# dfyz/osm-renderer

Measured on AMD Instinct MI355X. Metric: tiles/sec (256x256 z=15), higher is better.
Workload: dtype f64; 1 GPU; BASELINE.json configs[1]: batch of 1024 z=15 256x256 tiles per GPU, synthetic 50-poly/200-segment geometry per tile (SplitMix64, SURVEY.md 8(d)), lat/lon f64 input resident in HBM, RGBA8 framebuffers written to HBM; 2 batches in flight (step i on resident copy / stream i mod 2: the pre-pass of one batch overlaps the raster stage of the previous one); tiles_this_rank=1024, polygons_per_tile=50, polylines_per_tile=40, scale=1, named_config=True, collective=none (1 GPU), rccl_nranks_seen=1, batches_in_flight=2

## Files before the change

osm_renderer_amd/build.py:

```python
import os
import shutil
import subprocess

HERE = os.path.dirname(os.path.abspath(__file__))
CSRC = os.path.join(HERE, "csrc")
LIB = os.path.join(HERE, "libosmtile.so")
SOURCES = ["osmt_kernels.hip", "osmt_labels.hip", "osmt_glyphs.hip", "osmt_textplace.hip", "osmt_textshape.hip", "osmt_polylabel.hip", "osmt_styled.hip", "osmt_tilequery.hip", "osmt_tilelabels.hip", "osmt_arealabels.hip", "osmt_selmatch.hip", "osmt_labelbind.hip", "osmt_cascade.hip", "osmt_anchors.hip", "osmt_pngenc.hip", "osmt_api.cpp", "osmt_png.cpp"]
HEADERS = ["osmt_bitonic.h", "osmt_cascade_rule.h", "osmt_cascade_tables.h", "osmt_geom.h", "osmt_glyph.h", "osmt_internal.h", "osmt_list_slices.h", "osmt_numparse.h", "osmt_png_table.h", "osmt_prebin_roles.h", "osmt_project.h", "osmt_utf8.h", os.path.join("..", "host", "osmt_textplacer.hpp"),
           os.path.join("..", "host", "osmt_textshaper.hpp"),
           os.path.join("..", "..", "include", "osmtile.h")]
LIBS = ["-lz", "-ldl", "-lpthread", "-Wl,--no-undefined"]
FLAGS = ["--offload-arch=gfx950", "-O3", "-std=c++17", "-ffp-contract=off", "-fPIC", "-shared", "-Wall"]


def _hipcc():
    for cand in (shutil.which("hipcc"), "/opt/rocm/bin/hipcc"):
        if cand and os.path.exists(cand):
            return cand
    raise RuntimeError("hipcc not found; libosmtile.so cannot be built")


def needs_build():
    if not os.path.exists(LIB):
        return True
    t = os.path.getmtime(LIB)
    deps = [os.path.join(CSRC, s) for s in SOURCES + HEADERS]
    return any(os.path.getmtime(d) > t for d in deps)


def build_variant(name, defines):
    out = os.path.join(HERE, f"libosmtile_{name}.so")
    cmd = [_hipcc()] + FLAGS + [f"-D{d}" for d in defines] + ["-o", out] + [os.path.join(CSRC, s) for s in SOURCES] + LIBS
    subprocess.check_call(cmd)
    return out


def build(force=False, verbose=False):
    if not force and not needs_build():
        return LIB
    cmd = [_hipcc()] + FLAGS + ["-o", LIB] + [os.path.join(CSRC, s) for s in SOURCES] + LIBS
    if verbose:
        print(" ".join(cmd))
    subprocess.check_call(cmd)
    return LIB


if __name__ == "__main__":
    print(build(force=True, verbose=True))
```

osm_renderer_amd/csrc/osmt_api.cpp:

```cpp
#include <hip/hip_runtime.h>

#include <algorithm>
#include <chrono>
#include <atomic>
#include <cmath>
#include <cstdarg>
#include <cstdio>
#include <cstring>
#include <condition_variable>
#include <deque>
#include <functional>
#include <map>
#include <dlfcn.h>

#include <memory>
#include <mutex>
#include <thread>
#include <new>
#include <string>
#include <vector>

#include "../../include/osmtile.h"
#include "osmt_cascade_tables.h"
#include "osmt_geom.h"
// ... 55 lines not shown
        uint64_t tick;
    };
    std::mutex cache_mu;
    std::vector<cached_buf> cache;
    uint64_t cache_tick = 0;
    std::vector<hipStream_t> idle_streams;
    hipStream_t poison_stream = nullptr;
    std::vector<cached_buf> host_cache;
    std::vector<osmt_image_desc> images;
    std::vector<double> image_pool_host;
    osmt_image_desc* d_images = nullptr;
    double4* d_image_pool = nullptr;
    uint32_t d_n_images = 0;
    std::vector<void*> image_graveyard;
    bool images_dirty = false;
    std::vector<osmt_glyph_vertex> glyph_verts;
    std::vector<uint32_t> glyph_voff{0u};
    osmt_glyph_vertex* d_glyph_verts = nullptr;
    uint32_t* d_glyph_voff = nullptr;
    uint32_t d_n_glyphs = 0;
    bool glyphs_dirty = false;
    struct font_host {
        std::vector<osmt_cmap_entry> cmap;
        std::vector<int32_t> advance;
        std::vector<uint32_t> outline;
        std::vector<osmt_kern_pair> kern;
        osmt_font_desc view{};
        void* d_pool = nullptr;
        osmt_font_dev dev{};
    };
    std::vector<std::shared_ptr<font_host>> fonts;
    osmt_font_dev* d_fonts = nullptr;
    uint32_t d_n_fonts = 0;
    bool fonts_dirty = false;
    struct geodata_host {
        size_t n_nodes = 0, n_ways = 0, n_mps = 0;
        void* d_pool = nullptr;
        osmt_geo_dev dev{};
        void* d_index = nullptr;
        osmt_tq_index_dev ix{};
        void* d_node_index = nullptr;
        const uint32_t *d_node_off = nullptr, *d_node_refs = nullptr, *d_zero_off = nullptr;
        const uint64_t* d_node_gid = nullptr;
        const double2* d_factors = nullptr;
        void* d_tags = nullptr;
        osmt_sm_tags_dev tags{};
        size_t tags_string_bytes = 0, n_node_tags = 0, n_way_tags = 0;
    };
    std::vector<geodata_host> geodata;
    struct selectors_host {
        void* d_pool = nullptr;
        osmt_sm_sels_dev dev{};
        std::shared_ptr<const std::vector<uint8_t>> zooms;
    };
    std::vector<selectors_host> selectors;
    struct rules_host {
        void* d_pool = nullptr;
        osmt_cs_rules_dev dev{};
        uint32_t selectors_id = 0;
        std::shared_ptr<const std::vector<uint32_t>> key_off;
        std::shared_ptr<const std::vector<uint8_t>> key_bytes;
    };
    std::vector<rules_host> rules;
    uint32_t match_hash_bits = 32;
    struct bindings_host {
        uint32_t geodata_id = 0;
        uint8_t zoom_lo = 0, zoom_hi = 0;
        void* d_pool = nullptr;
        osmt_tq_bind_dev dev{};
    };
    std::vector<bindings_host> bindings;
    struct label_bindings_host {
        uint32_t geodata_id = 0;
        uint8_t zoom_lo = 0, zoom_hi = 0;
        void* d_pool = nullptr;
        osmt_tl_bind_dev dev{};
        size_t n_nodes = 0, n_bindings = 0, n_texts = 0, n_chars = 0;
    };
    std::vector<label_bindings_host> label_bindings;
    struct area_label_bindings_host {
        uint32_t geodata_id = 0;
        uint8_t zoom_lo = 0, zoom_hi = 0;
        void* d_pool = nullptr;
        osmt_al_bind_dev dev{};
        size_t n_ways = 0, n_mps = 0, n_way_bindings = 0, n_mp_bindings = 0, n_texts = 0, n_chars = 0;
    };
    std::vector<area_label_bindings_host> area_label_bindings;
    std::vector<osmt_label_style_rec> label_styles;
    osmt_label_style_rec* d_label_styles = nullptr;
    uint32_t* d_label_rank = nullptr;
    uint32_t d_n_label_styles = 0;
    bool label_styles_dirty = false;
    std::vector<osmt_style_rec> styles;
    std::vector<double> style_dashes;
    osmt_style_rec* d_styles = nullptr;
    uint32_t* d_style_rank = nullptr;
    double* d_style_dashes = nullptr;
    uint32_t d_n_styles = 0;
    bool styles_dirty = false;
    std::atomic<int> refs{1};
    void* comm = nullptr;
    uint32_t comm_rank = 0, comm_size = 0;
    unsigned long long* d_count = nullptr;
    uint32_t* err_page = nullptr;
    std::vector<uint16_t> err_free;
    struct arena_density {
        double groups_per_fill = 0.0, recs_per_vseg = 0.0;
        uint32_t uploads = 0;
    } density[OSMT_MAX_SCALE + 1];
    std::mutex co_mu;
    std::condition_variable co_cv;
    std::deque<struct coalesce_req*> co_queue;
    int co_in_flight = 0;
    uint64_t pl_stats[3] = {0, 0, 0};
};

struct osmt_scene {
    osmt_ctx* ctx = nullptr;
    uint32_t n_jobs = 0, n_ops = 0, n_rings = 0, n_pts = 0, n_dashes = 0, n_strokes = 0;
    uint32_t scale = 1, coord_kind = 0, n_blk = 0;
    char* d_base = nullptr;
    char* d_front = nullptr;
    size_t bytes = 0;
    osmt_tile_job* d_jobs = nullptr;
    osmt_op* d_ops = nullptr;
    osmt_ring* d_rings = nullptr;
    double* d_latlon = nullptr;
    uint32_t* d_node_refs = nullptr;
    int32_t* d_pts = nullptr;
    double* d_dashes = nullptr;
    uint32_t* d_pt_job = nullptr;
    uint32_t* d_op_aux = nullptr;
    osmt_opinfo* d_info = nullptr;
    osmt_stroke_aux* d_aux = nullptr;
    osmt_dash_seg* d_dseg = nullptr;
    uint32_t* d_submask = nullptr;
    uint32_t* d_op_blk = nullptr;
    uint32_t* d_op_vseg = nullptr;
    osmt_blk_bbox* d_blk = nullptr;
    uint32_t* d_op_job = nullptr;
    osmt_vseg* d_vseg = nullptr;
    unsigned long long* d_cursors = nullptr;
    uint32_t* d_cnt = nullptr;
    uint2* d_hdr = nullptr;
    osmt_ent* d_ent = nullptr;
    unsigned long long ent_cap = 0;
    uint32_t n_fill_ops = 0;
    uint32_t n_vsegs = 0;
    char* d_arena = nullptr;
    uint32_t* d_fmask = nullptr;
    osmt_srec* d_srec = nullptr;
    uint2* d_skey = nullptr;
    unsigned long long fmask_cap = 0, srec_cap = 0;
    std::vector<uint32_t> h_pt_job, h_op_aux, h_op_blk, h_op_vseg, h_op_job, h_lab_wide;
    std::vector<osmt_label_band> h_lab_bands;
    std::vector<osmt_labelinfo> h_lab_info;
    hipStream_t own_stream = nullptr;
    std::mutex use_mu;
    std::vector<std::pair<hipStream_t, hipEvent_t>> last_use;
    void* h_stage = nullptr;
    uint32_t* h_err = nullptr;
    uint32_t max_job_ops = 0;
    bool arena_guess = false;
    uint32_t n_labels = 0, n_label_segs = 0;
    char* d_lab_base = nullptr;
    osmt_labelinfo* d_lab = nullptr;
    uint32_t* d_job_label_off = nullptr;
    double* d_lab_segs = nullptr;
    double* d_lab_a = nullptr;
    double* d_lab_s_wide = nullptr;
    uint32_t* d_lab_wide = nullptr;
    osmt_label_band* d_lab_bands = nullptr;
    unsigned long long* d_lab_bits = nullptr;
    uint32_t n_lab_bands = 0;
    uint32_t n_lab_wide = 0;
    bool lab_cover_valid = false;
    uint32_t* d_lab_bitmap = nullptr;
    uint8_t* d_lab_ok = nullptr;
    uint32_t* d_lab_err = nullptr;
    osmt_tile_label* d_tile_labels = nullptr;
    uint32_t* d_tile_label_cnt = nullptr;
    osmt_glyph_instance* d_text_inst = nullptr;
    uint32_t n_text_inst = 0;
    osmt_text_glyph* d_text_glyphs = nullptr;
    uint32_t n_text_glyphs = 0;
    char* d_tq = nullptr;
    char* d_tq_areas_buf = nullptr;
    const osmt_styled_tile* d_tq_tiles = nullptr;
    const osmt_styled_area* d_tq_areas = nullptr;
    size_t n_tq_areas = 0;
    std::vector<osmt_query_tile> h_tq_tiles;
    uint32_t tq_geodata_id = 0;
    std::vector<osmt_label> h_tl_labels;
    std::vector<osmt_string_run> h_tl_runs;
    std::vector<uint32_t> h_tl_chars, h_tl_off;
    std::vector<osmt_label> h_al_labels;
    std::vector<osmt_string_run> h_al_runs;
    std::vector<uint32_t> h_al_chars, h_al_off;
    std::vector<int32_t> h_al_pts;
    std::vector<double> h_al_sincos;
    std::vector<osmt_area_anchor> h_al_declined;
};

namespace {

constexpr double OSMT_MAX_ABS_LAT = 85.06;
size_t cache_keep_bytes() {
    static const size_t v = [] {
        const char* e = getenv("OSMT_CACHE_GB");
        const long gb = e ? atol(e) : 32;
        return (size_t)std::min<long>(std::max<long>(gb, 0), 256) << 30;
    }();
    return v;
}

bool poison_alloc() {
    static const bool v = [] {
        const char* e = getenv("OSMT_POISON_ALLOC");
        return e && *e && *e != '0';
    }();
    return v;
}

hipError_t stream_acquire(osmt_ctx* ctx, hipStream_t* out);
void stream_release(osmt_ctx* ctx, hipStream_t st);

hipError_t dev_poison(osmt_ctx* ctx, void* p, size_t bytes) {
    hipStream_t st = nullptr;
    {
        std::lock_guard<std::mutex> lk(ctx->cache_mu);
        if (!ctx->poison_stream) {
            int lo = 0, hi = 0;
            (void)hipDeviceGetStreamPriorityRange(&lo, &hi);
            if (hipStreamCreateWithPriority(&ctx->poison_stream, hipStreamNonBlocking, hi) != hipSuccess) {
                (void)hipGetLastError();
                ctx->poison_stream = nullptr;
            }
        }
        st = ctx->poison_stream;
    }
    const bool pooled = st == nullptr;
    hipError_t e = pooled ? stream_acquire(ctx, &st) : hipSuccess;
    if (e != hipSuccess) return e;
    e = hipMemsetAsync(p, 0xA5, bytes, st);
    if (e == hipSuccess) e = hipStreamSynchronize(st);
    if (pooled) stream_release(ctx, st);
    return e;
}

hipError_t dev_alloc_raw(osmt_ctx* ctx, void** out, size_t bytes, size_t* got);

hipError_t dev_alloc(osmt_ctx* ctx, void** out, size_t bytes) {
    size_t got = 0;
    hipError_t e = dev_alloc_raw(ctx, out, bytes, &got);
    if (e == hipSuccess && poison_alloc()) e = dev_poison(ctx, *out, got);
    return e;
}

hipError_t dev_alloc_raw(osmt_ctx* ctx, void** out, size_t bytes, size_t* got) {
    bytes = align_up(bytes ? bytes : 1, (size_t)2 << 20);
    {
        std::lock_guard<std::mutex> lk(ctx->cache_mu);
        osmt_ctx::cached_buf* best = nullptr;
        for (auto& c : ctx->cache)
            if (!c.used && c.bytes >= bytes && c.bytes <= 2 * bytes && (!best || c.bytes < best->bytes)) best = &c;
        if (best) {
            best->used = true;
            best->tick = ++ctx->cache_tick;
            *out = best->p;
            *got = best->bytes;
            return hipSuccess;
        }
    }
    hipError_t e = hipMalloc(out, bytes);
    if (e == hipErrorOutOfMemory) {
        (void)hipGetLastError();
        std::lock_guard<std::mutex> lk(ctx->cache_mu);
        for (size_t i = 0; i < ctx->cache.size();) {
            if (!ctx->cache[i].used) {
                (void)hipFree(ctx->cache[i].p);
                ctx->cache.erase(ctx->cache.begin() + (long)i);
            } else {
                ++i;
            }
        }
        e = hipMalloc(out, bytes);
    }
    if (e != hipSuccess) return e;
    std::lock_guard<std::mutex> lk(ctx->cache_mu);
    ctx->cache.push_back({*out, bytes, true, ++ctx->cache_tick});
    *got = bytes;
    return hipSuccess;
}

hipError_t stream_acquire(osmt_ctx* ctx, hipStream_t* out) {
    {
        std::lock_guard<std::mutex> lk(ctx->cache_mu);
        if (!ctx->idle_streams.empty()) {
            *out = ctx->idle_streams.back();
            ctx->idle_streams.pop_back();
            return hipSuccess;
        }
    }
    return hipStreamCreateWithFlags(out, hipStreamNonBlocking);
}

// ... 347 lines not shown
        if (e != hipSuccess && first == hipSuccess) first = e;
    }
    return first;
}

int validate_coords_range(const osmt_batch* b, size_t lo, size_t hi) {
    if (b->coord_kind == OSMT_COORD_POINT_I32) {
        for (size_t i = 2 * lo; i < 2 * hi; ++i)
            if (b->points[i] > OSMT_COORD_LIMIT || b->points[i] < -OSMT_COORD_LIMIT)
                return fail(OSMT_UNSUPPORTED, "point %zu: |coordinate| > 2^28", i / 2);
    } else {
        const double* ll = b->coord_kind == OSMT_COORD_NODE_REF ? b->nodes : b->latlon;
        for (size_t i = lo; i < hi; ++i) {
            const double lat = ll[2 * i], lon = ll[2 * i + 1];
            if (!(std::fabs(lat) <= OSMT_MAX_ABS_LAT) || !(std::fabs(lon) <= 180.0))
                return fail(OSMT_UNSUPPORTED, "point %zu: (lat, lon) = (%g, %g) outside the Web-Mercator square (|lat| <= %g, |lon| <= 180)", i, lat,
                            lon, OSMT_MAX_ABS_LAT);
        }
    }
    return OSMT_OK;
}
size_t coord_count(const osmt_batch* b) { return b->coord_kind == OSMT_COORD_NODE_REF ? b->n_nodes : b->n_pts; }

int validate_batch_global(const osmt_batch* b) {
    if (!b) return fail(OSMT_INVALID_ARG, "batch is NULL");
    if (b->scale < 1 || b->scale > OSMT_MAX_SCALE) return fail(OSMT_INVALID_ARG, "scale %u not in 1..%u", b->scale, OSMT_MAX_SCALE);
    if (b->coord_kind != OSMT_COORD_LATLON_F64 && b->coord_kind != OSMT_COORD_POINT_I32 && b->coord_kind != OSMT_COORD_NODE_REF)
        return fail(OSMT_INVALID_ARG, "unknown coord_kind %u", b->coord_kind);
    if (b->n_jobs >= 0x7FFFFFFFull / 64 || b->n_ops >= 0xFFFFFFFFull || b->n_rings >= 0xFFFFFFFFull ||
        b->n_pts >= 0xFFFFFFFFull || b->n_dashes >= 0xFFFFFFFFull)
        return fail(OSMT_INVALID_ARG, "batch too large for 32-bit indices");
    if ((b->n_jobs && !b->jobs) || (b->n_ops && !b->ops) || (b->n_rings && !b->rings) || (b->n_dashes && !b->dashes))
        return fail(OSMT_INVALID_ARG, "NULL pool with non-zero count");
    if (b->n_pts) {
        if (b->coord_kind == OSMT_COORD_LATLON_F64 && !b->latlon) return fail(OSMT_INVALID_ARG, "latlon pool is NULL");
        if (b->coord_kind == OSMT_COORD_POINT_I32 && !b->points) return fail(OSMT_INVALID_ARG, "points pool is NULL");
        if (b->coord_kind == OSMT_COORD_NODE_REF) {
            if (!b->node_refs || !b->nodes) return fail(OSMT_INVALID_ARG, "node table / node_refs is NULL");
            if (b->n_nodes >= 0xFFFFFFFFull) return fail(OSMT_INVALID_ARG, "node table too large for 32-bit indices");
        }
    }
    struct range {
        uint64_t lo, hi;
        uint32_t job;
    };
    std::vector<range> ops, pts;
    ops.reserve(b->n_jobs);
    pts.reserve(b->n_jobs);
    for (size_t j = 0; j < b->n_jobs; ++j) {
        const osmt_tile_job& job = b->jobs[j];
        if (job.zoom > OSMT_MAX_ZOOM) return fail(OSMT_INVALID_ARG, "job %zu: zoom %u > MAX_ZOOM (src/tile.rs:5)", j, job.zoom);
        if ((size_t)job.op_off + job.n_ops > b->n_ops) return fail(OSMT_INVALID_ARG, "job %zu: op range out of bounds", j);
        if ((size_t)job.pt_off + job.n_pts > b->n_pts) return fail(OSMT_INVALID_ARG, "job %zu: point range out of bounds", j);
        if (job.n_ops) ops.push_back({job.op_off, (uint64_t)job.op_off + job.n_ops, (uint32_t)j});
        if (job.n_pts) pts.push_back({job.pt_off, (uint64_t)job.pt_off + job.n_pts, (uint32_t)j});
    }
    auto by_lo = [](const range& x, const range& y) { return x.lo < y.lo; };
    std::sort(ops.begin(), ops.end(), by_lo);
    uint64_t next = 0;
    for (const range& r : ops) {
        if (r.lo < next)
            return fail(OSMT_INVALID_ARG, "job %u: op %llu also belongs to another job (op ranges must not overlap)", r.job, (unsigned long long)r.lo);
        if (r.lo > next)
            return fail(OSMT_INVALID_ARG, "op %llu is not covered by any job (the jobs' op ranges must partition the op pool)", (unsigned long long)next);
        next = r.hi;
    }
    if (next != b->n_ops)
        return fail(OSMT_INVALID_ARG, "op %llu is not covered by any job (the jobs' op ranges must partition the op pool)", (unsigned long long)next);
    std::sort(pts.begin(), pts.end(), by_lo);
    for (size_t i = 1; i < pts.size(); ++i)
        if (pts[i].lo < pts[i - 1].hi) return fail(OSMT_INVALID_ARG, "the point ranges of two jobs overlap at point %llu", (unsigned long long)pts[i].lo);
    return OSMT_OK;
}

int validate_job(const osmt_batch* b, size_t j, bool with_coords = true) {
    const osmt_tile_job& job = b->jobs[j];
    for (uint32_t k = 0; k < job.n_ops; ++k) {
        const osmt_op& op = b->ops[job.op_off + k];
        if (op.kind > OSMT_OP_STROKE) return fail(OSMT_INVALID_ARG, "job %zu op %u: unknown kind %u", j, k, op.kind);
        if (op.kind == OSMT_OP_NONE) continue;
        if ((size_t)op.ring_off + op.n_rings > b->n_rings) return fail(OSMT_INVALID_ARG, "job %zu op %u: ring range out of bounds", j, k);
        for (uint32_t r = 0; r < op.n_rings; ++r) {
            const osmt_ring& ring = b->rings[op.ring_off + r];
            if (ring.first_pt < job.pt_off || (size_t)ring.first_pt + ring.n_pts > (size_t)job.pt_off + job.n_pts)
                return fail(OSMT_INVALID_ARG, "job %zu op %u ring %u: points outside the job's pool range", j, k, r);
        }
        if (!(op.opacity >= 0.0) || !(op.opacity <= 4503599627370496.0))
            return fail(OSMT_INVALID_ARG, "job %zu op %u: opacity must be in [0, 2^52]", j, k);
        if (op.kind == OSMT_OP_STROKE) {
            if (!std::isfinite(op.width)) return fail(OSMT_INVALID_ARG, "job %zu op %u: width not finite", j, k);
            if (std::fabs(op.width) > 65536.0) return fail(OSMT_UNSUPPORTED, "job %zu op %u: |width| > 65536 px", j, k);
            if (op.cap > OSMT_CAP_SQUARE) return fail(OSMT_INVALID_ARG, "job %zu op %u: unknown cap", j, k);
            if (op.has_dashes) {
                if (op.n_dashes == 0) return fail(OSMT_INVALID_ARG, "job %zu op %u: empty dash list", j, k);
                if (op.n_dashes > OSMT_MAX_DASHES) return fail(OSMT_UNSUPPORTED, "job %zu op %u: more than %u dashes", j, k, OSMT_MAX_DASHES);
                if ((size_t)op.dashes_off + op.n_dashes > b->n_dashes) return fail(OSMT_INVALID_ARG, "job %zu op %u: dash range out of bounds", j, k);
            }
        }
    }
    if (b->coord_kind == OSMT_COORD_NODE_REF) {
        for (size_t i = job.pt_off; i < (size_t)job.pt_off + job.n_pts; ++i)
            if (b->node_refs[i] >= b->n_nodes) return fail(OSMT_INVALID_ARG, "point %zu: node reference %u out of range", i, b->node_refs[i]);
        return OSMT_OK;
    }
    return with_coords ? validate_coords_range(b, job.pt_off, (size_t)job.pt_off + job.n_pts) : OSMT_OK;
}

int validate_nodes(const osmt_batch* b, size_t lo, size_t hi) {
    return b->coord_kind == OSMT_COORD_NODE_REF ? validate_coords_range(b, lo, hi) : OSMT_OK;
}

int validate_batch(const osmt_batch* b, bool with_coords = true) {
    int rc = validate_batch_global(b);
    for (size_t j = 0; rc == OSMT_OK && j < b->n_jobs; ++j) rc = validate_job(b, j, with_coords);
    if (rc == OSMT_OK && with_coords) rc = validate_nodes(b, 0, b->n_nodes);
    return rc;
}

osmt_prepass_args prepass_args(const osmt_scene* sc, bool sizing) {
    osmt_prepass_args a;
    memset(&a, 0, sizeof a);
    a.jobs = sc->d_jobs;
    a.n_jobs = sc->n_jobs;
    a.ops = sc->d_ops;
    a.n_ops = sc->n_ops;
    a.rings = sc->d_rings;
    a.pts = reinterpret_cast<const int2*>(sc->d_pts);
    a.dashes = sc->d_dashes;
    a.op_aux = sc->d_op_aux;
    a.op_job = sc->d_op_job;
    a.op_blk = sc->d_op_blk;
    a.op_vseg = sc->d_op_vseg;
    a.vseg = sc->d_vseg;
    a.n_vsegs = sc->n_vsegs;
    a.max_job_ops = sc->max_job_ops;
    a.fold_max_ops = sc->n_jobs <= OSMT_FOLD_MAX_JOBS ? OSMT_FOLD_MAX_OPS : 0u;
    a.scale = sc->scale;
    a.sub_rows = OSMT_TILE_SIZE * sc->scale / OSMT_SUB_H;
    a.info = sc->d_info;
    a.aux = sc->d_aux;
    a.dseg = sc->d_dseg;
    a.blk = sc->d_blk;
    a.submask = sc->d_submask;
    a.cursors = sc->d_cursors;
    a.cnt = sc->d_cnt;
    a.hdr = sc->d_hdr;
    a.ent = sc->d_ent;
    a.ent_cap = sizing ? 0ull : sc->ent_cap;
    a.fmask = sc->d_fmask;
    a.srec = sc->d_srec;
    a.skey = sc->d_skey;
    a.fmask_cap = sizing ? 0ull : sc->fmask_cap;
    a.srec_cap = sizing ? 0ull : sc->srec_cap;
    a.err = sizing ? nullptr : sc->h_err;
    return a;
}

int render_impl(osmt_ctx* ctx, osmt_scene* sc, uint32_t stages, void* d_out, size_t stride, bool f64, void* stream,
                uint32_t first_job = 0, uint32_t n_range = 0) {
    if (!ctx || !sc || sc->ctx != ctx) return fail(OSMT_INVALID_ARG, "bad ctx/scene");
    HIP_TRY(hipSetDevice(ctx->device));
    hipStream_t st = (hipStream_t)stream;
    const uint32_t W = OSMT_TILE_SIZE * sc->scale;
    if ((stages & 4u) && !d_out) return fail(OSMT_INVALID_ARG, "output pointer is NULL");
    const bool rgb8 = (stages & 32u) != 0u;
    if ((stages & 4u) && !f64 && !rgb8 && stride < (size_t)W * W * 4) return fail(OSMT_INVALID_ARG, "out_tile_stride_bytes < W*H*4");
    if ((stages & 4u) && rgb8 && (f64 || stride < (size_t)W * W * 3 || (stride & 3u) || ((uintptr_t)d_out & 3u)))
        return fail(OSMT_INVALID_ARG, "RGB8 output: tile stride below W*H*3 or not a multiple of 4");
    bool zeroed = false;
    if ((stages & 1u) && sc->coord_kind != OSMT_COORD_POINT_I32) {
        const osmt_prepass_args pa = prepass_args(sc, false);
        zeroed = (stages & 2u) != 0u && sc->n_pts != 0u;
        HIP_TRY(osmt_launch_project(sc->d_jobs, sc->d_pt_job, sc->d_latlon, sc->coord_kind == OSMT_COORD_NODE_REF ? sc->d_node_refs : nullptr,
                                    sc->n_pts, (double)sc->scale, sc->d_pts, st, zeroed ? reinterpret_cast<uint32_t*>(pa.cursors) : nullptr,
                                    zeroed ? osmt_prepass_zero_words(pa) : 0));
    }
    if (stages & 2u) HIP_TRY(osmt_launch_prepass(prepass_args(sc, false), st, zeroed));
    const bool want_labels = sc->n_labels && !f64;
    if (want_labels && ((stages & 8u) || ((stages & 4u) && !(stages & 16u)))) {
        int rc = sync_images(ctx, nullptr);
        if (rc != OSMT_OK) return rc;
        osmt_label_launch ll;
        memset(&ll, 0, sizeof ll);
        ll.info = sc->d_lab;
        ll.n_labels = sc->n_labels;
        ll.n_jobs = sc->n_jobs;
        ll.scale = sc->scale;
        ll.n_wide = sc->n_lab_wide;
        ll.bands = sc->d_lab_bands;
        ll.n_bands = sc->n_lab_bands;
        ll.job_label_off = sc->d_job_label_off;
        ll.segs = sc->d_lab_segs;
        ll.wide = sc->d_lab_wide;
        ll.plane_a = sc->d_lab_a;
        ll.cell_bits = sc->d_lab_bits;
        ll.plane_s_wide = sc->d_lab_s_wide;
        ll.bitmap = sc->d_lab_bitmap;
        ll.ok = sc->d_lab_ok;
        ll.err = sc->d_lab_err;
        ll.tile_labels = sc->d_tile_labels;
        ll.tile_label_cnt = sc->d_tile_label_cnt;
        HIP_TRY(osmt_launch_labels(ll, st));
        sc->lab_cover_valid = true;
    }
    if (stages & 4u) {
        image_snapshot img;
        int rc = sync_images(ctx, &img);
        if (rc != OSMT_OK) return rc;
        if (first_job > sc->n_jobs || n_range > sc->n_jobs - first_job) return fail(OSMT_INVALID_ARG, "tile range out of bounds");
        const uint32_t n_render = n_range ? n_range : sc->n_jobs - first_job;
        osmt_raster_args a;
        memset(&a, 0, sizeof a);
        a.jobs = sc->d_jobs + first_job;
        a.n_jobs = n_render;
        a.scale = sc->scale;
        a.aux = sc->d_aux;
        a.dseg = sc->d_dseg;
        {
            const uint32_t Wt = OSMT_TILE_SIZE * sc->scale;
            a.hdr = sc->d_hdr + (size_t)first_job * (Wt / OSMT_SUB_W) * (Wt / OSMT_SUB_H);
        }
        a.ent = sc->d_ent;
        a.fmask = sc->d_fmask;
        a.srec = sc->d_srec;
        a.skey = sc->d_skey;
        a.info = sc->d_info;
        a.submask = sc->d_submask;
        a.fold_max_ops = sc->n_jobs <= OSMT_FOLD_MAX_JOBS ? OSMT_FOLD_MAX_OPS : 0u;
        a.images = img.desc;
        a.image_pool = img.pool;
        a.n_images = img.n;
        a.out = d_out;
        a.out_tile_stride = stride;
        a.out_rgb8 = rgb8 ? 1u : 0u;
        if (want_labels) {
            a.labels.info = sc->d_lab;
            a.labels.n_labels = sc->n_labels;
            a.labels.job_label_off = sc->d_job_label_off + first_job;
            a.labels.tile_labels = sc->d_tile_labels;
            a.labels.tile_label_cnt = sc->d_tile_label_cnt + first_job;
            a.labels.plane = sc->d_lab_a;
        }
        HIP_TRY(osmt_launch_raster(a, f64, st));
    }
    HIP_TRY(scene_mark_use(sc, st));
    return OSMT_OK;
}

}

extern "C" {

uint32_t osmt_version(void) { return (1u << 16) | 1u; }

const char* osmt_last_error(void) { return g_last_error.c_str(); }

static int osmt_create_body(const osmt_config* cfg, osmt_ctx** out_ctx) {
    if (!out_ctx) return fail(OSMT_INVALID_ARG, "out_ctx is NULL");
    *out_ctx = nullptr;
    int n = 0;
    hipError_t e = hipGetDeviceCount(&n);
    if (e != hipSuccess || n <= 0)
        return fail(OSMT_NO_DEVICE, "no HIP device available (%s); this library has no CPU path",
                    e == hipSuccess ? "device count 0" : hipGetErrorString(e));
    const int dev = cfg ? cfg->device : 0;
    if (dev < 0 || dev >= n) return fail(OSMT_INVALID_ARG, "device %d out of range (0..%d)", dev, n - 1);
    HIP_TRY(hipSetDevice(dev));
    osmt_ctx* c = new (std::nothrow) osmt_ctx();
    if (!c) return fail(OSMT_OOM, "out of host memory");
    c->device = dev;
    *out_ctx = c;
    return OSMT_OK;
}

int osmt_create(const osmt_config* cfg, osmt_ctx** out_ctx) {
    return guarded([&] { return osmt_create_body(cfg, out_ctx); });
}

void osmt_destroy(osmt_ctx* ctx) {
    if (!ctx) return;
    ctx_release(ctx);
}

static int osmt_register_image_body(osmt_ctx* ctx, const uint8_t* rgba8, uint32_t width, uint32_t height, uint32_t* out_id) {
    if (!ctx || !rgba8 || !out_id) return fail(OSMT_INVALID_ARG, "NULL argument");
    if (width == 0 || height == 0) return fail(OSMT_INVALID_ARG, "empty image");
    std::lock_guard<std::mutex> lk(ctx->mu);
    osmt_image_desc d;
    d.offset = ctx->image_pool_host.size() / 4;
    d.width = width;
    d.height = height;
    const size_t n = (size_t)width * height;
    ctx->image_pool_host.reserve(ctx->image_pool_host.size() + 4 * n);
    for (size_t i = 0; i < n; ++i) {
        const double a = (double)rgba8[4 * i + 3] / 255.0;
        ctx->image_pool_host.push_back(a * ((double)rgba8[4 * i + 0] / 255.0));
        ctx->image_pool_host.push_back(a * ((double)rgba8[4 * i + 1] / 255.0));
        ctx->image_pool_host.push_back(a * ((double)rgba8[4 * i + 2] / 255.0));
        ctx->image_pool_host.push_back(a);
    }
    *out_id = (uint32_t)ctx->images.size();
    ctx->images.push_back(d);
    ctx->images_dirty = true;
    return OSMT_OK;
}

int osmt_register_image(osmt_ctx* ctx, const uint8_t* rgba8, uint32_t width, uint32_t height, uint32_t* out_id) {
    return guarded([&] { return osmt_register_image_body(ctx, rgba8, width, height, out_id); });
}

static int osmt_register_glyphs_body(osmt_ctx* ctx, const osmt_glyph_vertex* v, const uint32_t* voff, uint32_t n, uint32_t* out_first) {
    if (!ctx || !voff || !out_first) return fail(OSMT_INVALID_ARG, "NULL argument");
    if (voff[0] != 0) return fail(OSMT_INVALID_ARG, "vertex_off[0] must be 0");
    for (uint32_t i = 0; i < n; ++i)
        if (voff[i] > voff[i + 1]) return fail(OSMT_INVALID_ARG, "vertex_off is not monotonic at glyph %u", i);
    const uint32_t nv = voff[n];
    if (nv && !v) return fail(OSMT_INVALID_ARG, "NULL vertex pool");
    for (uint32_t k = 0; k < nv; ++k)
        if (v[k].type < OSMT_GLYPH_MOVE_TO || v[k].type > OSMT_GLYPH_CURVE_TO)
            return fail(OSMT_INVALID_ARG, "glyph vertex %u: type %u is not MoveTo / LineTo / CurveTo", k, (unsigned)v[k].type);
    std::lock_guard<std::mutex> lk(ctx->mu);
    const size_t base = ctx->glyph_verts.size();
    if (base + nv >= 0xFFFFFFFFull || ctx->glyph_voff.size() + n >= 0xFFFFFFFFull) return fail(OSMT_INVALID_ARG, "glyph table too large");
    *out_first = (uint32_t)(ctx->glyph_voff.size() - 1);
    ctx->glyph_verts.insert(ctx->glyph_verts.end(), v, v + nv);
    for (uint32_t i = 1; i <= n; ++i) ctx->glyph_voff.push_back((uint32_t)(base + voff[i]));
    ctx->glyphs_dirty = true;
    return OSMT_OK;
}

int osmt_register_glyphs(osmt_ctx* ctx, const osmt_glyph_vertex* v, const uint32_t* vertex_off, uint32_t n_glyphs, uint32_t* out_first_id) {
    return guarded([&] { return osmt_register_glyphs_body(ctx, v, vertex_off, n_glyphs, out_first_id); });
}

static int osmt_register_font_body(osmt_ctx* ctx, const osmt_font_desc* font, uint32_t* out_id) {
    if (!ctx || !out_id) return fail(OSMT_INVALID_ARG, "NULL argument");
    std::lock_guard<std::mutex> lk(ctx->mu);
    std::string why;
    const int rc = osmt::validate_font(font, ctx->glyph_voff.size() - 1, &why);
    if (rc != OSMT_OK) return fail(rc, "%s", why.c_str());
    if (ctx->fonts.size() + 1 >= 0xFFFFFFFFull) return fail(OSMT_INVALID_ARG, "font table too large");
    auto f = std::make_shared<osmt_ctx::font_host>();
    f->cmap.assign(font->cmap, font->cmap + font->n_cmap);
    f->advance.assign(font->advance, font->advance + font->n_glyphs);
    f->outline.assign(font->outline_id, font->outline_id + font->n_glyphs);
    if (font->n_kern) f->kern.assign(font->kern, font->kern + font->n_kern);
    f->view = *font;
    f->view.cmap = f->cmap.data();
    f->view.advance = f->advance.data();
    f->view.outline_id = f->outline.data();
    f->view.kern = f->kern.empty() ? nullptr : f->kern.data();
    *out_id = (uint32_t)ctx->fonts.size();
    ctx->fonts.push_back(std::move(f));
    ctx->fonts_dirty = true;
    return OSMT_OK;
}

int osmt_register_font(osmt_ctx* ctx, const osmt_font_desc* font, uint32_t* out_font_id) {
    return guarded([&] { return osmt_register_font_body(ctx, font, out_font_id); });
}

static std::vector<const osmt_font_desc*> font_views(osmt_ctx* ctx, std::vector<std::shared_ptr<osmt_ctx::font_host>>* keep) {
    {
        std::lock_guard<std::mutex> lk(ctx->mu);
        *keep = ctx->fonts;
    }
    std::vector<const osmt_font_desc*> v;
    for (const auto& f : *keep) v.push_back(&f->view);
    return v;
}

static int scene_size_arenas(osmt_ctx* ctx, osmt_scene* s, size_t n_fills, bool allow_guess) {
    const size_t W = (size_t)OSMT_TILE_SIZE * s->scale;
    const size_t nsub = (W / OSMT_SUB_W) * (W / OSMT_SUB_H);
    unsigned long long groups = (unsigned long long)n_fills * nsub, recs = (unsigned long long)s->n_vsegs * nsub;
    const unsigned long long worst_bytes = groups * 64ull + recs * (sizeof(osmt_srec) + 8ull) +
                                           osmt_list_layout_make(s->n_jobs, ((unsigned long long)n_fills + s->n_strokes) * nsub).total * sizeof(osmt_ent);
    bool guessed = false;
    if (worst_bytes > ((unsigned long long)32 << 20) && allow_guess && s->h_err != nullptr) {
        std::lock_guard<std::mutex> lk(ctx->cache_mu);
        osmt_ctx::arena_density& d = ctx->density[s->scale];
        if (d.uploads != 0 && (d.uploads & 63u) != 0 && d.groups_per_fill > 0.0 && d.recs_per_vseg > 0.0) {
            const unsigned long long g = (unsigned long long)(d.groups_per_fill * 1.25 * (double)n_fills) + 4096ull;
            const unsigned long long r = (unsigned long long)(d.recs_per_vseg * 1.25 * (double)s->n_vsegs) + 4096ull;
            groups = std::min(groups, g);
            recs = std::min(recs, r);
            guessed = true;
            ++d.uploads;
        }
    }
    s->arena_guess = guessed;
    if (worst_bytes > ((unsigned long long)32 << 20) && !guessed) {
        hipStream_t st = s->own_stream;
        if (s->coord_kind != OSMT_COORD_POINT_I32)
            HIP_TRY(osmt_launch_project(s->d_jobs, s->d_pt_job, s->d_latlon, s->coord_kind == OSMT_COORD_NODE_REF ? s->d_node_refs : nullptr,
                                        s->n_pts, (double)s->scale, s->d_pts, st));
        HIP_TRY(osmt_launch_prepass(prepass_args(s, true), st));
        unsigned long long totals[2] = {0ull, 0ull};
        HIP_TRY(hipMemcpyAsync(totals, s->d_cursors, sizeof totals, hipMemcpyDeviceToHost, st));
        HIP_TRY(hipStreamSynchronize(st));
        groups = totals[0];
        recs = totals[1];
        std::lock_guard<std::mutex> lk(ctx->cache_mu);
        osmt_ctx::arena_density& d = ctx->density[s->scale];
        if (n_fills) d.groups_per_fill = std::max(d.groups_per_fill * 0.98, (double)groups / (double)n_fills);
        if (s->n_vsegs) d.recs_per_vseg = std::max(d.recs_per_vseg * 0.98, (double)recs / (double)s->n_vsegs);
        if (d.groups_per_fill <= 0.0) d.groups_per_fill = 1e-9;
        if (d.recs_per_vseg <= 0.0) d.recs_per_vseg = 1e-9;
        ++d.uploads;
    }
    if (groups >= OSMT_MAX_FILL_GROUPS)
        return fail(OSMT_UNSUPPORTED, "scene needs %llu fill groups (>= 2^28 = %llu, the most a list entry's 32-bit word index reaches): split the batch",
                    groups, (unsigned long long)OSMT_MAX_FILL_GROUPS);
    if (groups >= 0xFFFFFFFFull || recs >= 0xFFFFFFFFull)
        return fail(OSMT_UNSUPPORTED, "scene needs %llu fill groups / %llu stroke records (> 2^32): split the batch", groups, recs);
    size_t off = 0;
    auto carve = [&](size_t bytes) {
        const size_t o = off;
        off = align_up(off + bytes, 256);
        return o;
    };
    unsigned long long ents = std::min<unsigned long long>(groups + recs, ((unsigned long long)n_fills + s->n_strokes) * nsub);
    if (ents >= 0xFFFFFFFFull) return fail(OSMT_UNSUPPORTED, "scene needs %llu list entries (> 2^32): split the batch", ents);
    const size_t o_f = carve((size_t)(groups + 1) * 64);
    const size_t o_r = carve((size_t)(recs + 1) * sizeof(osmt_srec));
    const size_t o_k = carve((size_t)(recs + 1) * 8);
    const osmt_list_layout lay = osmt_list_layout_make(s->n_jobs, ents + 1);
    const size_t o_e = carve((size_t)lay.total * sizeof(osmt_ent));
    hipError_t e = dev_alloc(ctx, (void**)&s->d_arena, off + 256);
    if (e != hipSuccess) {
        s->d_arena = nullptr;
        return fail(e == hipErrorOutOfMemory ? OSMT_OOM : OSMT_HIP_ERROR, "hipMalloc(%zu) for the pre-pass arenas failed: %s", off, hipGetErrorString(e));
    }
    s->d_fmask = (uint32_t*)(s->d_arena + o_f);
    s->d_srec = (osmt_srec*)(s->d_arena + o_r);
    s->d_skey = (uint2*)(s->d_arena + o_k);
    s->d_ent = (osmt_ent*)(s->d_arena + o_e);
    s->ent_cap = ents + 1;
    static const bool trace_arenas = getenv("OSMT_TRACE_UPLOAD") != nullptr;
    if (trace_arenas)
        fprintf(stderr, "osmt arenas: %u tiles, fill groups %llu, stroke records %llu, list entries %llu in %u slice(s) of %llu (+ overflow): "
                        "list arena %.1f MB of %.1f MB%s\n", s->n_jobs, groups, recs, ents + 1, lay.n_slices, lay.slice_cap,
                (double)lay.total * sizeof(osmt_ent) / 1e6, (double)off / 1e6, guessed ? " (guessed)" : "");
    s->fmask_cap = groups + 1;
    s->srec_cap = recs + 1;
    return OSMT_OK;
}

struct scene_back {
    size_t o_info, o_aux, o_dseg, o_submask, o_blk, o_vseg, o_cursors, o_hdr;
};
static scene_back scene_carve_back(size_t& off, size_t n_jobs, size_t n_ops, size_t n_strokes, size_t n_blk, size_t n_vsegs, uint32_t scale) {
    auto carve = [&](size_t bytes) {
        const size_t o = off;
        off = align_up(off + bytes, 256);
        return o;
    };
    scene_back k;
    k.o_info = carve(n_ops * sizeof(osmt_opinfo));
    k.o_aux = carve((size_t)(n_strokes + 1) * sizeof(osmt_stroke_aux));
    k.o_dseg = carve((size_t)(n_strokes + 1) * OSMT_MAX_DASH_SEGS * sizeof(osmt_dash_seg));
    const size_t sub_rows = (size_t)OSMT_TILE_SIZE * scale / OSMT_SUB_H;
    k.o_submask = carve(n_ops * sub_rows * 4);
    k.o_blk = carve((n_blk + 1) * sizeof(osmt_blk_bbox));
    k.o_vseg = carve((n_vsegs + 1) * sizeof(osmt_vseg));
    const size_t n_sub = ((size_t)OSMT_TILE_SIZE * scale / OSMT_SUB_W) * sub_rows;
    k.o_cursors = carve((osmt_list_cursor_word0(n_jobs * n_sub) + OSMT_LIST_CURSOR_WORDS) * 4);
    k.o_hdr = carve(n_jobs * n_sub * sizeof(uint2));
    return k;
}
static void scene_point_back(osmt_scene* s, char* rbase, const scene_back& k) {
    s->d_info = (osmt_opinfo*)(rbase + k.o_info);
    s->d_aux = (osmt_stroke_aux*)(rbase + k.o_aux);
    s->d_dseg = (osmt_dash_seg*)(rbase + k.o_dseg);
    s->d_submask = (uint32_t*)(rbase + k.o_submask);
    s->d_blk = (osmt_blk_bbox*)(rbase + k.o_blk);
    s->d_vseg = (osmt_vseg*)(rbase + k.o_vseg);
    s->d_cursors = (unsigned long long*)(rbase + k.o_cursors);
    s->d_cnt = (uint32_t*)(rbase + k.o_cursors + 32);
    s->d_hdr = (uint2*)(rbase + k.o_hdr);
}

static int scene_upload_impl(osmt_ctx* ctx, const osmt_batch* b, osmt_scene** out_scene, hipStream_t st, bool trusted = false,
                             bool allow_guess = false) {
    if (!ctx || !out_scene) return fail(OSMT_INVALID_ARG, "NULL argument");
    *out_scene = nullptr;
    const bool big = b && coord_count(b) >= ((size_t)1 << 16);
    size_t off = 0;
    auto carve = [&](size_t bytes) {
        const size_t o = off;
        off = align_up(off + bytes, 256);
        return o;
    };
    const bool ll = b && b->coord_kind == OSMT_COORD_LATLON_F64;
    const bool nr = b && b->coord_kind == OSMT_COORD_NODE_REF;
    size_t o_jobs = 0, o_ops = 0, o_rings = 0, o_latlon = 0, o_refs = 0, o_pts = 0, o_dashes = 0, o_ptjob = 0, o_opaux = 0, o_opblk = 0, o_opvseg = 0,
           o_opjob = 0, front_bytes = 0;
    if (b) {
        o_jobs = carve(b->n_jobs * sizeof(osmt_tile_job));
        o_ops = carve(b->n_ops * sizeof(osmt_op));
        o_rings = carve(b->n_rings * sizeof(osmt_ring));
        o_latlon = carve(ll ? b->n_pts * 16 : nr ? b->n_nodes * 16 : 0);
        o_refs = carve(nr ? b->n_pts * 4 : 0);
        o_pts = carve(b->n_pts * 8);
        o_dashes = carve((b->n_dashes + 1) * 8);
        o_ptjob = carve(b->n_pts * 4);
        o_opaux = carve(b->n_ops * 4);
        o_opblk = carve(b->n_ops * 4);
        o_opvseg = carve(b->n_ops * 4);
        o_opjob = carve(b->n_ops * 4);
        front_bytes = off;
    }
    const bool split = big && st != nullptr && front_bytes > STAGE_MAX_BYTES;
    int rc = OSMT_OK;
    if (!trusted) rc = split ? validate_batch_global(b) : validate_batch(b, !big);
    if (rc != OSMT_OK) return rc;
    HIP_TRY(hipSetDevice(ctx->device));
    struct coord_check {
        std::vector<std::thread> th;
        std::vector<int> rc;
        std::vector<std::string> msg;
        int join() {
            for (auto& t : th)
                if (t.joinable()) t.join();
            for (size_t i = 0; i < rc.size(); ++i)
                if (rc[i] != OSMT_OK) return fail(rc[i], "%s", msg[i].c_str());
            return OSMT_OK;
        }
        void wait() {
            for (auto& t : th)
                if (t.joinable()) t.join();
        }
        ~coord_check() { wait(); }
    } cc;
    const unsigned n_coord_thr = (big && !trusted) ? (coord_count(b) >= ((size_t)1 << 19) ? 2u : 1u) : 0u;
    cc.rc.assign(n_coord_thr + (split ? 2u : 0u), OSMT_OK);
    cc.msg.resize(n_coord_thr + (split ? 2u : 0u));
    if (big && !trusted) {
        const size_t n = coord_count(b);
        const unsigned n_thr = n_coord_thr;
        for (unsigned t = 0; t < n_thr; ++t) {
            const size_t lo = n * t / n_thr, hi = n * (t + 1) / n_thr;
            try {
                cc.th.emplace_back([&cc, b, t, lo, hi] {
                    cc.rc[t] = guarded([&] { return validate_coords_range(b, lo, hi); });
                    if (cc.rc[t] != OSMT_OK) cc.msg[t] = osmt_last_error();
                });
            } catch (...) {
                cc.rc[t] = validate_coords_range(b, lo, hi);
                if (cc.rc[t] != OSMT_OK) cc.msg[t] = osmt_last_error();
            }
        }
    }

    char* d_front = nullptr;
    struct front_guard {
        osmt_ctx* ctx;
        coord_check* cc;
        hipStream_t st;
        char* p = nullptr;
        ~front_guard() {
            if (!p) return;
            cc->wait();
            (void)hipStreamSynchronize(st);
            dev_free(ctx, p);
        }
    } fg{ctx, &cc, st ? st : nullptr};
    if (split) {
        hipError_t fe = dev_alloc(ctx, (void**)&d_front, front_bytes + 256);
        if (fe != hipSuccess) {
            cc.wait();
            return fail(fe == hipErrorOutOfMemory ? OSMT_OOM : OSMT_HIP_ERROR, "hipMalloc(%zu) failed: %s", front_bytes, hipGetErrorString(fe));
        }
        fg.p = d_front;
        auto copy_user_arrays = [&cc, ctx, b, st, d_front, ll, nr, o_jobs, o_ops, o_rings, o_latlon, o_refs, o_pts, o_dashes](unsigned slot, bool coords) {
            cc.rc[slot] = guarded([&] {
                HIP_TRY(hipSetDevice(ctx->device));
                auto put = [&](size_t o, const void* src, size_t bytes) -> hipError_t {
                    return bytes ? hipMemcpyAsync(d_front + o, src, bytes, hipMemcpyHostToDevice, st) : hipSuccess;
                };
                if (!coords) {
                    HIP_TRY(put(o_jobs, b->jobs, b->n_jobs * sizeof(osmt_tile_job)));
                    HIP_TRY(put(o_ops, b->ops, b->n_ops * sizeof(osmt_op)));
                    HIP_TRY(put(o_rings, b->rings, b->n_rings * sizeof(osmt_ring)));
                    HIP_TRY(put(o_dashes, b->dashes, b->n_dashes * 8));
                } else {
                    if (ll) HIP_TRY(put(o_latlon, b->latlon, b->n_pts * 16));
                    if (nr) HIP_TRY(put(o_latlon, b->nodes, b->n_nodes * 16));
                    if (nr) HIP_TRY(put(o_refs, b->node_refs, b->n_pts * 4));
                    if (!ll && !nr) HIP_TRY(put(o_pts, b->points, b->n_pts * 8));
                }
// ... 6263 lines not shown
```

osm_renderer_amd/csrc/osmt_internal.h:

```cpp
#ifndef OSMT_INTERNAL_H
#define OSMT_INTERNAL_H

#include <hip/hip_runtime.h>
#include <stdint.h>

#include "../../include/osmtile.h"
#include "osmt_glyph.h"
#include "osmt_list_slices.h"

#define OSMT_SUB_W 32
#ifndef OSMT_SUB_H_LOG2
#define OSMT_SUB_H_LOG2 4
#endif
#define OSMT_SUB_H (1 << OSMT_SUB_H_LOG2)

#define OSMT_MAX_DASH_SEGS 10

struct osmt_dash_seg {
    double start_from, start_to, end_from, end_to, opacity_mul;
    double orig_a, orig_b;
    double r_start, r_end;
};

struct osmt_cap_seg {
    int32_t p1x, p1y, p2x, p2y;
    int32_t valid;
    uint32_t cand_off;
    double denom;
};

struct alignas(64) osmt_stroke_aux {
    double half_width;
    double hlw0, ff0, ft0, fd0, mul0;
    double rfd0;
    int32_t main_n_segs;
    int32_t main_has_orig;
    double main_total_len;
    double main_r_total;
    int32_t caps_has_orig;
    int32_t _pad;
    osmt_dash_seg caps_seg;
};
static_assert(sizeof(osmt_stroke_aux) == 192, "three 64-byte lines");

struct osmt_opinfo {
    int32_t x0, y0, x1, y1;
    uint32_t aux;
    uint32_t n_edges;
    uint32_t first_pt;
    uint32_t n_rings;
    uint8_t kind, cap, color[3], _pad[3];
    uint32_t arena_off;
    uint32_t rec_cap;
    union {
        struct {
            uint32_t fill_geom;
            uint32_t image_id;
        };
        double stroke_ft;
    };
    double opacity;
};
static_assert(sizeof(osmt_opinfo) == 64, "osmt_opinfo must be one 64-byte record");

struct alignas(16) osmt_srec {
    int32_t p1x, p1y, p2x, p2y;
    double traveled;
    double denom;
    double rdenom;
    int32_t k_lo0, k_lo1;
    int32_t m_lo0, m_lo1;
    uint16_t k_n0, k_n1, n_x0, n_x1;
};
static_assert(sizeof(osmt_srec) == 64, "osmt_srec is one 64-byte line: four 16-byte stores by k_stroke_bin, four loads by k_raster");

struct alignas(16) osmt_vseg {
    int32_t p1x, p1y, p2x, p2y;
    double trav;
    double den, rden;
    uint32_t cand_off;
    uint32_t vop;
};
static_assert(sizeof(osmt_vseg) == 48, "three 16-byte words");

struct osmt_blk_bbox {
    int32_t x0, y0, x1, y1;
};

struct alignas(16) osmt_ent {
    uint32_t arena;
    uint32_t kind_color;
    double opacity;
    uint32_t aux;
    uint32_t nv;
    uint32_t stage;
    uint32_t _pad;
};
static_assert(sizeof(osmt_ent) == 32, "osmt_ent is two 16-byte loads");

struct osmt_image_desc {
    uint64_t offset;
    uint32_t width, height;
};

struct osmt_label_seg {
    double x0, y0;
    double slope, slope_recip;
    double y_min, y_max;
    double sign;
    int32_t yf, yl;
};
static_assert(sizeof(osmt_label_seg) == 64, "osmt_label_seg must be one 64-byte record");

struct osmt_labelinfo {
    uint32_t seg_off, n_segs;
    int32_t ry0, ry1;
    int32_t cx0;
    uint32_t cols;
    uint64_t plane_off;
    int32_t icon_x, icon_y;
    uint32_t icon_w, icon_h;
    uint64_t icon_off;
    uint8_t has_text, color[3];
    uint32_t wide_off;
};
static_assert(sizeof(osmt_labelinfo) == 64, "osmt_labelinfo must be one 64-byte record");

#ifndef OSMT_LABEL_LDS_CELLS
#define OSMT_LABEL_LDS_CELLS 576
#endif

struct osmt_tile_label {
    int16_t x0, y0, x1, y1;
    uint32_t label;
    uint32_t _pad;
};

struct osmt_label_band {
    uint32_t label, rbase;
};
__host__ __device__ static inline uint32_t osmt_label_band_rows(uint32_t cols) {
    const uint32_t r = OSMT_LABEL_LDS_CELLS / cols;
    return r < 64u ? r : 64u;
}
__host__ __device__ static inline uint32_t osmt_label_band_words(uint32_t cols) { return (osmt_label_band_rows(cols) * cols + 63u) / 64u; }

struct osmt_label_launch {
    const osmt_labelinfo* info;
    const osmt_label_band* bands;
    uint32_t n_bands;
    uint32_t n_labels, n_jobs, scale, n_wide;
    const uint32_t* job_label_off;
    const double* segs;
    const uint32_t* wide;
    double* plane_a;
    unsigned long long* cell_bits;
    double* plane_s_wide;
    uint32_t* bitmap;
    uint8_t* ok;
    uint32_t* err;
    osmt_tile_label* tile_labels;
    uint32_t* tile_label_cnt;
};

struct osmt_label_args {
    const osmt_labelinfo* info;
    uint32_t n_labels;
    const uint32_t* job_label_off;
    const osmt_tile_label* tile_labels;
    const uint32_t* tile_label_cnt;
    const double* plane;
};

struct osmt_glyph_pass {
    const osmt_glyph_vertex* verts;
    const uint32_t* voff;
    const osmt_glyph_instance* inst;
    const uint32_t* pair_inst;
    const uint32_t* pair_label;
    uint32_t n_pairs;
    int32_t W;
    osmt_label_extent* sum;
    uint32_t* pair_cnt;
    uint32_t* pair_base;
    uint32_t* blk;
    uint32_t* err;
    double* segs;
    uint32_t n_segs;
};

#define OSMT_FOLD_MAX_OPS 128u
#define OSMT_FOLD_MAX_JOBS 64u

struct osmt_raster_args {
    const osmt_tile_job* jobs;
    uint32_t n_jobs;
    uint32_t scale;
    const osmt_stroke_aux* aux;
    const osmt_dash_seg* dseg;
    const uint2* hdr;
    const osmt_ent* ent;
    const uint32_t* fmask;
    const osmt_srec* srec;
    uint32_t fold_max_ops;
    uint32_t _pad1;
    const osmt_opinfo* info;
    const uint32_t* submask;
    const uint2* skey;
    const osmt_image_desc* images;
    const double4* image_pool;
    uint32_t n_images;
    uint32_t out_rgb8;
    void* out;
    size_t out_tile_stride;
    osmt_label_args labels;
};

struct osmt_prepass_args {
    const osmt_tile_job* jobs;
    uint32_t n_jobs;
    const osmt_op* ops;
    uint32_t n_ops;
    const osmt_ring* rings;
    const int2* pts;
    const double* dashes;
    const uint32_t* op_aux;
    const uint32_t* op_job;
    const uint32_t* op_blk;
    const uint32_t* op_vseg;
    uint32_t n_vsegs;
    uint32_t scale;
    uint32_t sub_rows;
    uint32_t max_job_ops;
    uint32_t fold_max_ops;
    osmt_opinfo* info;
    osmt_stroke_aux* aux;
    osmt_dash_seg* dseg;
    osmt_blk_bbox* blk;
    uint32_t* submask;
    osmt_vseg* vseg;
    unsigned long long* cursors;
    uint32_t* cnt;
    uint2* hdr;
    osmt_ent* ent;
    unsigned long long ent_cap;
    uint32_t* fmask;
    osmt_srec* srec;
    uint2* skey;
    unsigned long long fmask_cap, srec_cap;
    uint32_t* err;
};
#define OSMT_PREPASS_ERR_FILL_ARENA 1u
#define OSMT_PREPASS_ERR_STROKE_ARENA 2u
#define OSMT_PREPASS_ERR_LIST_ARENA 4u

struct osmt_pl_req {
    uint32_t ring_off, n_rings;
    uint32_t keep_off;
    uint32_t _pad;
    double scale;
};
static_assert(sizeof(osmt_pl_req) == 24, "osmt_pl_req");

#define OSMT_PL_GLOBAL_CELLS OSMT_LABEL_MAX_CELLS
#define OSMT_PL_CELL_DOUBLES 5u
#define OSMT_PL_ERR_HEAP 1u
#define OSMT_PL_ERR_KEEP 2u
#define OSMT_PL_ERR_GRID 4u
#define OSMT_PL_ERR_LIST 8u
#define OSMT_PL_ERR_TIER1 16u
#define OSMT_PL_ERR_TIER2 32u
#define OSMT_PL_MAX_SLOTS 64u

struct osmt_polylabel_args {
    const osmt_pl_req* req;
    uint32_t n_req;
    const osmt_ring* rings;
    uint32_t n_rings;
    const double2* pts;
    uint32_t* keep;
    osmt_label_position* out;
    uint32_t* over;
    uint32_t* cnt;
    double* ws;
    uint32_t n_slots;
};
hipError_t osmt_launch_polylabel(const osmt_polylabel_args& a, hipStream_t st);

hipError_t osmt_launch_project(const osmt_tile_job* jobs, const uint32_t* pt_job, const double* latlon, const uint32_t* refs,
                               uint32_t n_pts, double scale, int32_t* pts, hipStream_t st, uint32_t* zero = nullptr, size_t n_zero = 0);
size_t osmt_prepass_zero_words(const osmt_prepass_args& a);
hipError_t osmt_launch_ptjob(const osmt_tile_job* jobs, uint32_t n_jobs, uint32_t* pt_job, uint32_t n_pts, hipStream_t st);
hipError_t osmt_launch_project_single(const double* latlon, uint32_t n, uint32_t zoom, uint32_t tx, uint32_t ty,
                                      double scale, int32_t* pts, hipStream_t st);
hipError_t osmt_launch_prepass(const osmt_prepass_args& a, hipStream_t st, bool zeroed = false);
hipError_t osmt_launch_raster(const osmt_raster_args& a, bool out_f64, hipStream_t st);
hipError_t osmt_launch_labels(const osmt_label_launch& a, hipStream_t st);
hipError_t osmt_launch_glyph_count(const osmt_glyph_pass& a, uint32_t n_labels, hipStream_t st);
hipError_t osmt_launch_glyph_emit(const osmt_glyph_pass& a, hipStream_t st);
struct osmt_text_pass {
    const osmt_label* labels;
    uint32_t n_labels;
    const osmt_text_run* runs;
    const osmt_text_glyph* glyphs;
    const int32_t* way_pts;
    const double* way_sincos;
    osmt_glyph_instance* inst;
};
hipError_t osmt_launch_text_place(const osmt_text_pass& a, hipStream_t st);
struct osmt_font_dev {
    const osmt_cmap_entry* cmap;
    const int32_t* advance;
    const uint32_t* outline;
    const osmt_kern_pair* kern;
    uint32_t n_cmap, n_kern, n_glyphs, _pad;
};
struct osmt_shape_pass {
    const osmt_label* labels;
    const uint32_t* label_font;
    const uint32_t* pair_inst;
    const uint32_t* pair_label;
    uint32_t n_pairs;
    const uint32_t* chars;
    const osmt_font_dev* fonts;
    osmt_text_glyph* out;
};
hipError_t osmt_launch_text_shape(const osmt_shape_pass& a, hipStream_t st);
struct osmt_geo_dev {
    const double* nodes;
    const uint64_t* way_gid;
    const uint64_t* mp_gid;
    const uint32_t* way_off;
    const uint32_t* poly_off;
    const uint32_t* mp_off;
    const uint32_t* mp_polys;
    const uint32_t* idx;
    const uint2* mp_sum;
};

enum { OSMT_SQ_OPS = 0, OSMT_SQ_RINGS, OSMT_SQ_REFS, OSMT_SQ_DASHES, OSMT_SQ_STROKES, OSMT_SQ_BLOCKS, OSMT_SQ_VSEGS, OSMT_SQ_N };
#define OSMT_STYLED_TOTALS (OSMT_SQ_N + 1)

struct osmt_styled_pass {
    osmt_geo_dev geo;
    const osmt_style_rec* styles;
    const uint32_t* style_rank;
    const double* style_dashes;
    const osmt_styled_tile* tiles;
    const uint32_t* tile_base;
    const osmt_styled_area* areas;
    uint32_t n_tiles;
    uint32_t n_elems;
    uint32_t scale, use_caps;
    ulonglong2* keys;
    uint32_t* sorted;
    uint32_t* pre;
    unsigned long long* blk;
    unsigned long long* totals;
    osmt_tile_job* jobs;
    osmt_op* ops;
    osmt_ring* rings;
    uint32_t* refs;
    double* dashes;
    uint32_t *op_job, *op_aux, *op_blk, *op_vseg;
    uint32_t* ring_src;
    uint32_t n_rings, n_refs;
};
hipError_t osmt_launch_styled_count(const osmt_styled_pass& a, hipStream_t st);
hipError_t osmt_launch_styled_emit(const osmt_styled_pass& a, hipStream_t st);

struct osmt_tq_index_dev {
    const uint32_t* col_x;
    const uint32_t* col_first;
    const uint32_t* tile_y;
    const uint32_t* way_off;
    const uint32_t* ways;
    const uint32_t* mp_off;
    const uint32_t* mps;
    uint32_t n_cols, n_tiles;
};
struct osmt_tq_bind_dev {
    const uint32_t *way_off, *way_styles, *mp_off, *mp_styles;
};
enum {
    OSMT_TQ_ITEMS = 0,
    OSMT_TQ_WAYS,
    OSMT_TQ_MPS,
    OSMT_TQ_MAX_CAND,
    OSMT_TQ_OVER_CAND,
    OSMT_TQ_AREAS,
    OSMT_TQ_MAX_AREAS,
    OSMT_TQ_OVER_AREAS,
    OSMT_TQ_N
};
// ... 329 lines not shown
```

osm_renderer_amd/csrc/osmt_kernels.hip:

```cpp
#include <hip/hip_runtime.h>
#include <stdint.h>

#include "../../include/osmtile.h"
#include "osmt_geom.h"
#include "osmt_internal.h"
#include "osmt_prebin_roles.h"
#include "osmt_project.h"

namespace {

__device__ __forceinline__ uint32_t f64_as_u8(double v) {
#if defined(__HIP_DEVICE_COMPILE__) && !defined(OSMT_V_PLAIN_CVT)
    uint32_t r;
    asm("v_cvt_u32_f64 %0, %1" : "=v"(r) : "v"(v));
    return min(r, 255u);
#else
    return (uint32_t)(int32_t)fmin(fmax(v, 0.0), 255.0);
#endif
}

__device__ __forceinline__ uint32_t wave_incl_scan(uint32_t x) {
    x += (uint32_t)__builtin_amdgcn_update_dpp(0, (int)x, 0x111, 0xF, 0xF, false);
    x += (uint32_t)__builtin_amdgcn_update_dpp(0, (int)x, 0x112, 0xF, 0xF, false);
    x += (uint32_t)__builtin_amdgcn_update_dpp(0, (int)x, 0x114, 0xF, 0xF, false);
    x += (uint32_t)__builtin_amdgcn_update_dpp(0, (int)x, 0x118, 0xF, 0xF, false);
    x += (uint32_t)__builtin_amdgcn_update_dpp(0, (int)x, 0x142, 0xA, 0xF, false);
    x += (uint32_t)__builtin_amdgcn_update_dpp(0, (int)x, 0x143, 0xC, 0xF, false);
    return x;
}

__global__ __launch_bounds__(256) void k_project(const osmt_tile_job* __restrict__ jobs,
                                                 const uint32_t* __restrict__ pt_job,
                                                 const double2* __restrict__ latlon, const uint32_t* __restrict__ refs,
                                                 uint32_t n_pts, double scale, int2* __restrict__ pts, uint32_t* __restrict__ zero,
                                                 uint32_t n_zero) {
    const uint32_t i = blockIdx.x * 256u + threadIdx.x;
    if (i < n_zero) zero[i] = 0u;
    if (i >= n_pts) return;
    const uint32_t j = pt_job[i];
    if (j == 0xFFFFFFFFu) {
        pts[i] = make_int2(0, 0);
        return;
    }
    const osmt_tile_job job = jobs[j];
    const double2 ll = latlon[refs ? refs[i] : i];
    int32_t x, y;
    project_point(ll.x, ll.y, job.zoom, job.x, job.y, scale, &x, &y);
    pts[i] = make_int2(x, y);
}

__global__ __launch_bounds__(256) void k_ptjob(const osmt_tile_job* __restrict__ jobs, uint32_t* __restrict__ pt_job) {
    const osmt_tile_job job = jobs[blockIdx.x];
    for (uint32_t i = threadIdx.x; i < job.n_pts; i += 256u) pt_job[job.pt_off + i] = blockIdx.x;
}

__global__ __launch_bounds__(256) void k_project_single(const double2* __restrict__ latlon, uint32_t n, uint32_t zoom,
                                                        uint32_t tx, uint32_t ty, double scale,
                                                        int2* __restrict__ pts) {
    const uint32_t i = blockIdx.x * 256u + threadIdx.x;
    if (i >= n) return;
    const double2 ll = latlon[i];
    int32_t x, y;
    project_point(ll.x, ll.y, zoom, tx, ty, scale, &x, &y);
    pts[i] = make_int2(x, y);
}

__device__ __forceinline__ double point_dist(int32_t ax, int32_t ay, int32_t bx, int32_t by) {
    const double dx = (double)(ax - bx);
    const double dy = (double)(ay - by);
    return sqrt(dx * dx + dy * dy);
}

__device__ __forceinline__ int2 push_away_from(int2 self, int2 other, double by) {
    const double dist = point_dist(self.x, self.y, other.x, other.y);
    const double k = by / dist;
    int2 r;
    r.x = self.x + f64_as_i32(round((double)(self.x - other.x) * k));
    r.y = self.y + f64_as_i32(round((double)(self.y - other.y) * k));
    return r;
}

__device__ __forceinline__ int compute_segments(double hlw, const double* __restrict__ dashes, int n_dashes, int cap, osmt_dash_seg* segs,
                                                int max_out, double* total_len) {
    double len_before = 0.0;
    int n = 0;
    for (int it = 0; it <= n_dashes; ++it) {
        const int idx = (it < n_dashes) ? it : 0;
        const double dash = dashes[idx];
        double start = len_before;
        if (idx != 0 || n == 0) len_before += dash;
        if (idx % 2 != 0) continue;
        double end = start + dash;
        osmt_dash_seg s;
        s.orig_a = start;
        s.orig_b = end;
        if (cap == OSMT_CAP_SQUARE || cap == OSMT_CAP_ROUND) {
            start -= hlw;
            end += hlw;
        }
        const double midpoint = (start + end) / 2.0;
        s.start_from = fmin(start - 0.5, midpoint - 1.0);
        s.start_to = fmin(start + 0.5, midpoint);
        s.end_from = fmax(end - 0.5, midpoint);
        s.end_to = fmax(end + 0.5, midpoint + 1.0);
        s.opacity_mul = fmin(end - start, 1.0);
        s.r_start = 1.0 / (s.start_to - s.start_from);
        s.r_end = 1.0 / (s.end_to - s.end_from);
        if (n < max_out) segs[n] = s;
        ++n;
    }
    *total_len = len_before;
    return n;
}

struct SubWindow {
    int32_t sx0, sx1, sy0, sy1;
};
__device__ __forceinline__ double stroke_ft(double half_width) { return fmax(fabs(half_width) + 0.5, 1.0); }
__device__ __forceinline__ SubWindow vseg_window(int32_t p1x, int32_t p1y, int32_t p2x, int32_t p2y, double len, double ft,
                                                 int32_t n_sub_x, int32_t n_sub_y) {
    const int32_t dx = abs(p2x - p1x), dy = abs(p2y - p1y);
    const bool swap = dx > dy;
    const osmt_run_reach rr = osmt_reach_of(swap ? dy : dx, swap ? dx : dy, len, ft);
    const int32_t rx = swap ? rr.c_extra : rr.t_extra, ry = swap ? rr.t_extra : rr.c_extra;
    SubWindow w;
    w.sx0 = max((min(p1x, p2x) - rx) >> 5, 0);
    w.sx1 = min((max(p1x, p2x) + rx) >> 5, n_sub_x - 1);
    w.sy0 = max((min(p1y, p2y) - ry) >> OSMT_SUB_H_LOG2, 0);
    w.sy1 = min((max(p1y, p2y) + ry) >> OSMT_SUB_H_LOG2, n_sub_y - 1);
    return w;
}
__device__ __forceinline__ uint32_t window_count(const SubWindow& w) {
    if (w.sx0 > w.sx1 || w.sy0 > w.sy1) return 0u;
    return (uint32_t)(w.sx1 - w.sx0 + 1) * (uint32_t)(w.sy1 - w.sy0 + 1);
}

#ifndef OSMT_V_OPINFO_THREADS
#define OSMT_V_OPINFO_THREADS 64
#endif
constexpr uint32_t OPINFO_THREADS = OSMT_V_OPINFO_THREADS;
static_assert(OPINFO_THREADS == 64 || OPINFO_THREADS == 32 || OPINFO_THREADS == 16, "the wave scans read their totals from the last active lane");
#ifndef OSMT_V_OPINFO_WAVES
#define OSMT_V_OPINFO_WAVES 8
#endif
constexpr uint32_t OPINFO_WAVES = OSMT_V_OPINFO_WAVES;
static_assert(OPINFO_WAVES == 1 || OPINFO_THREADS == 64, "several waves per workgroup: whole waves");
__global__ __launch_bounds__(OPINFO_THREADS * OPINFO_WAVES) void k_opinfo(const osmt_prepass_args a) {
    const uint32_t op_lane = threadIdx.x % OPINFO_THREADS, op_wave = threadIdx.x / OPINFO_THREADS;
    const uint32_t wblk = blockIdx.x * OPINFO_WAVES + op_wave;
    const uint32_t o_raw = wblk * OPINFO_THREADS + op_lane;
    const bool live = o_raw < a.n_ops;
    const uint32_t o = live ? o_raw : a.n_ops - 1u;
    osmt_op op = a.ops[o];
    if (!live) op.kind = OSMT_OP_NONE;
    const osmt_ring* __restrict__ rings = a.rings;
    const int2* __restrict__ pts = a.pts;
    const uint32_t sub_rows = a.sub_rows;
    {
        const size_t w_first = min((size_t)a.n_ops, (size_t)wblk * OPINFO_THREADS) * sub_rows;
        const size_t w_end = min((size_t)a.n_ops, (size_t)(wblk + 1u) * OPINFO_THREADS) * sub_rows;
        for (size_t i = w_first + op_lane; i < w_end; i += OPINFO_THREADS) a.submask[i] = 0u;
    }
    osmt_opinfo oi;
    oi.x0 = oi.y0 = INT32_MAX;
    oi.x1 = oi.y1 = INT32_MIN;
    oi.aux = a.op_aux[o];
    oi.n_edges = 0;
    oi.first_pt = op.kind != OSMT_OP_NONE && op.n_rings ? rings[op.ring_off].first_pt : 0u;
    oi.n_rings = op.kind != OSMT_OP_NONE ? op.n_rings : 0u;
    oi.kind = op.kind;
    oi.cap = op.cap;
    oi.color[0] = op.color[0];
    oi.color[1] = op.color[1];
    oi.color[2] = op.color[2];
    oi._pad[0] = oi._pad[1] = oi._pad[2] = 0;
    oi.arena_off = 0;
    oi.rec_cap = 0;
    oi.fill_geom = 0;
    oi.image_id = op.image_id;
    oi.opacity = op.opacity;
    const bool none = op.kind == OSMT_OP_NONE;
    if (none) op.n_rings = 0u;
    const int32_t W = (int32_t)(OSMT_TILE_SIZE * a.scale);
    const int32_t n_sub_y = (int32_t)sub_rows, n_sub_x = W / OSMT_SUB_W;
    const bool is_stroke = op.kind == OSMT_OP_STROKE;
    uint32_t n_edges = 0;
    for (uint32_t r = 0; r < op.n_rings; ++r) {
        const uint32_t np = rings[op.ring_off + r].n_pts;
        if (np >= 2u) n_edges += np - 1u;
    }
    oi.n_edges = n_edges;
    const double hw = op.width / 2.0;
    const double ft = stroke_ft(hw);
    const bool caps = is_stroke && (op.cap == OSMT_CAP_ROUND || op.cap == OSMT_CAP_SQUARE);
    osmt_cap_seg c0 = {0, 0, 0, 0, 0, 0u, 1.0}, c1 = {0, 0, 0, 0, 0, 0u, 1.0};
    unsigned long long cand = 0ull;
    double traveled = 0.0;
    uint32_t seen = 0;
    const uint32_t blk_off = a.op_blk[o];
    const uint32_t vbase = a.op_vseg[o];
    uint32_t cur_blk = 0xFFFFFFFFu;
    osmt_blk_bbox bb = {INT32_MAX, INT32_MAX, INT32_MIN, INT32_MIN};
    for (uint32_t r = 0; r < op.n_rings; ++r) {
        const osmt_ring ring = rings[op.ring_off + r];
        const int2* __restrict__ rp = pts + ring.first_pt;
        const uint32_t np = ring.n_pts;
        const int2 zero2 = make_int2(0, 0);
        int2 q0 = np > 0u ? rp[0] : zero2, q1 = np > 1u ? rp[1] : zero2, q2 = np > 2u ? rp[2] : zero2, q3 = np > 3u ? rp[3] : zero2;
        int2 prev = zero2;
        for (uint32_t i = 0; i < np; ++i) {
            const int2 p = q0;
            q0 = q1;
            q1 = q2;
            q2 = q3;
            q3 = (i + 4u < np) ? rp[i + 4u] : zero2;
            oi.x0 = min(oi.x0, p.x);
            oi.x1 = max(oi.x1, p.x);
            oi.y0 = min(oi.y0, p.y);
            oi.y1 = max(oi.y1, p.y);
            if (i > 0u) {
                ++seen;
                if (blk_off != 0xFFFFFFFFu) {
                    const uint32_t b_ = (seen - 1u) >> 6;
                    if (b_ != cur_blk) {
                        if (cur_blk != 0xFFFFFFFFu) a.blk[blk_off + cur_blk] = bb;
                        cur_blk = b_;
                        bb = {INT32_MAX, INT32_MAX, INT32_MIN, INT32_MIN};
                    }
                    bb.x0 = min(bb.x0, min(prev.x, p.x));
                    bb.y0 = min(bb.y0, min(prev.y, p.y));
                    bb.x1 = max(bb.x1, max(prev.x, p.x));
                    bb.y1 = max(bb.y1, max(prev.y, p.y));
                }
                if (is_stroke) {
                    const double len = point_dist(prev.x, prev.y, p.x, p.y);
                    const uint32_t e = vbase + seen - 1u;
                    {
                        osmt_vseg vs;
                        vs.p1x = prev.x; vs.p1y = prev.y; vs.p2x = p.x; vs.p2y = p.y;
                        vs.trav = traveled;
                        vs.den = len;
                        vs.rden = 1.0 / len;
                        vs.cand_off = (uint32_t)min(cand, 0xFFFFFFFFull);
                        vs.vop = o;
                        a.vseg[e] = vs;
                    }
                    traveled += len;
                    if (!(prev.x == p.x && prev.y == p.y)) {
                        cand += window_count(vseg_window(prev.x, prev.y, p.x, p.y, len, ft, n_sub_x, n_sub_y));
                        if (caps && seen == 1u) {
                            const int2 ce = push_away_from(prev, p, hw);
                            c0 = {prev.x, prev.y, ce.x, ce.y, 1, 0u, point_dist(ce.x, ce.y, prev.x, prev.y)};
                        }
                        if (caps && seen == n_edges) {
                            const int2 ce = push_away_from(p, prev, hw);
                            c1 = {p.x, p.y, ce.x, ce.y, 1, 0u, point_dist(ce.x, ce.y, p.x, p.y)};
                        }
                    }
                }
            }
            prev = p;
        }
    }
    if (cur_blk != 0xFFFFFFFFu) a.blk[blk_off + cur_blk] = bb;
    unsigned long long want_f = 0ull, want_s = 0ull;
    uint32_t fill_geom_ok = 0u;
    if (is_stroke) {
        if (c0.valid && (c0.p1x != c0.p2x || c0.p1y != c0.p2y)) {
            c0.cand_off = (uint32_t)min(cand, 0xFFFFFFFFull);
            cand += window_count(vseg_window(c0.p1x, c0.p1y, c0.p2x, c0.p2y, c0.denom, ft, n_sub_x, n_sub_y));
        }
        if (c1.valid && (c1.p1x != c1.p2x || c1.p1y != c1.p2y)) {
            c1.cand_off = (uint32_t)min(cand, 0xFFFFFFFFull);
            cand += window_count(vseg_window(c1.p1x, c1.p1y, c1.p2x, c1.p2y, c1.denom, ft, n_sub_x, n_sub_y));
        }
        if (caps) {
            const osmt_cap_seg* cs[2] = {&c0, &c1};
#pragma unroll
            for (int i = 0; i < 2; ++i) {
                const uint32_t e = vbase + n_edges + (uint32_t)i;
                const bool ok = cs[i]->valid != 0;
                osmt_vseg vs;
                vs.p1x = ok ? cs[i]->p1x : 0; vs.p1y = ok ? cs[i]->p1y : 0; vs.p2x = ok ? cs[i]->p2x : 0; vs.p2y = ok ? cs[i]->p2y : 0;
                vs.trav = 0.0;
                vs.den = cs[i]->denom;
                vs.rden = 1.0 / cs[i]->denom;
                vs.cand_off = cs[i]->cand_off;
                vs.vop = o | 0x80000000u;
                a.vseg[e] = vs;
            }
        }
        osmt_stroke_aux sv;
        sv.half_width = hw;
        sv.hlw0 = sqrt(hw * hw - 0.0 * 0.0);
        sv.ff0 = fmax(sv.hlw0 - 0.5, 0.0);
        sv.ft0 = fmax(sv.hlw0 + 0.5, 1.0);
        sv.fd0 = sv.ft0 - sv.ff0;
        sv.rfd0 = 1.0 / sv.fd0;
        sv.mul0 = fmin(2.0 * sv.hlw0, 1.0);
        const int cap_for_dashes = op.use_caps_for_dashes ? op.cap : OSMT_CAP_NONE;
        sv.main_n_segs = 0;
        sv.main_has_orig = 0;
        sv.main_total_len = 0.0;
        sv.main_r_total = 0.0;
        if (op.has_dashes) {
            sv.main_n_segs = compute_segments(hw, a.dashes + op.dashes_off, (int)op.n_dashes, cap_for_dashes,
                                              a.dseg + (size_t)oi.aux * OSMT_MAX_DASH_SEGS, OSMT_MAX_DASH_SEGS, &sv.main_total_len);
            sv.main_has_orig = (cap_for_dashes == OSMT_CAP_ROUND) ? 1 : 0;
            sv.main_r_total = 1.0 / sv.main_total_len;
        }
        const double zero = 0.0;
        double caps_total;
        (void)compute_segments(hw, &zero, 1, op.cap, &sv.caps_seg, 1, &caps_total);
        sv.caps_has_orig = (op.cap == OSMT_CAP_ROUND) ? 1 : 0;
        sv._pad = 0;
        a.aux[oi.aux] = sv;
        if (cand > 0xFFFFFFFFull) cand = 0xFFFFFFFFull;
        oi.rec_cap = (uint32_t)cand;
        oi.stroke_ft = ft;
        want_s = cand;
    } else if (!none) {
        const int32_t ylo = max(oi.y0 + 1, 0), yhi = min(oi.y1, W - 1);
        const int32_t xlo = max(oi.x0, 0), xhi = min(oi.x1, W - 1);
        if (oi.x0 <= oi.x1 && ylo <= yhi && xlo <= xhi) {
            const uint32_t sr0 = (uint32_t)(ylo >> OSMT_SUB_H_LOG2), nsr = (uint32_t)(yhi >> OSMT_SUB_H_LOG2) - sr0 + 1u;
            const uint32_t c0 = (uint32_t)(xlo >> 5), ncols = (uint32_t)(xhi >> 5) - c0 + 1u;
            want_f = (unsigned long long)nsr * ncols;
            fill_geom_ok = sr0 | (c0 << 8) | (ncols << 16) | (nsr << 24);
        }
    }
    {
        const uint32_t lane = op_lane;
        const uint32_t f = (uint32_t)want_f;
        const uint32_t s_lo = (uint32_t)want_s & 0xFFFFu, s_hi = (uint32_t)(want_s >> 16);
        const uint32_t f_incl = wave_incl_scan(f);
        const unsigned long long s_incl = ((unsigned long long)wave_incl_scan(s_hi) << 16) + wave_incl_scan(s_lo);
        const uint32_t f_tot = (uint32_t)__builtin_amdgcn_readlane((int)f_incl, OPINFO_THREADS - 1);
        const unsigned long long s_tot = ((unsigned long long)(uint32_t)__builtin_amdgcn_readlane((int)(uint32_t)(s_incl >> 32), OPINFO_THREADS - 1) << 32) |
                                         (uint32_t)__builtin_amdgcn_readlane((int)(uint32_t)s_incl, OPINFO_THREADS - 1);
        unsigned long long f_base = 0ull, s_base = 0ull;
        if (OPINFO_WAVES == 1u) {
            if (lane == 0u) {
                if (f_tot) f_base = atomicAdd(&a.cursors[0], (unsigned long long)f_tot);
                if (s_tot) s_base = atomicAdd(&a.cursors[1], s_tot);
            }
        } else {
            __shared__ unsigned long long s_tot_f[OPINFO_WAVES], s_tot_s[OPINFO_WAVES];
            if (lane == 0u) {
                s_tot_f[op_wave] = f_tot;
                s_tot_s[op_wave] = s_tot;
            }
            __syncthreads();
            if (threadIdx.x == 0u) {
                unsigned long long bf = 0ull, bs = 0ull;
                for (uint32_t w = 0; w < OPINFO_WAVES; ++w) {
                    bf += s_tot_f[w];
                    bs += s_tot_s[w];
                }
                bf = bf ? atomicAdd(&a.cursors[0], bf) : 0ull;
                bs = bs ? atomicAdd(&a.cursors[1], bs) : 0ull;
                for (uint32_t w = 0; w < OPINFO_WAVES; ++w) {
                    const unsigned long long tf = s_tot_f[w], ts = s_tot_s[w];
                    s_tot_f[w] = bf;
                    s_tot_s[w] = bs;
                    bf += tf;
                    bs += ts;
                }
            }
            __syncthreads();
            if (lane == 0u) {
                f_base = s_tot_f[op_wave];
                s_base = s_tot_s[op_wave];
            }
        }
        f_base = ((unsigned long long)(uint32_t)__builtin_amdgcn_readfirstlane((int)(uint32_t)(f_base >> 32)) << 32) |
                 (uint32_t)__builtin_amdgcn_readfirstlane((int)(uint32_t)f_base);
        s_base = ((unsigned long long)(uint32_t)__builtin_amdgcn_readfirstlane((int)(uint32_t)(s_base >> 32)) << 32) |
                 (uint32_t)__builtin_amdgcn_readfirstlane((int)(uint32_t)s_base);
        if (want_s) {
            const unsigned long long off = s_base + (s_incl - want_s);
            oi.arena_off = (uint32_t)off;
            if (a.srec_cap && off + want_s > a.srec_cap) {
                oi.rec_cap = 0;
                if (a.err) *(volatile uint32_t*)a.err = OSMT_PREPASS_ERR_STROKE_ARENA;
            }
        }
        if (want_f) {
            const unsigned long long off = f_base + (f_incl - f);
            oi.arena_off = (uint32_t)off;
            if (!(a.fmask_cap && off + want_f > a.fmask_cap))
                oi.fill_geom = fill_geom_ok;
            else if (a.err)
                *(volatile uint32_t*)a.err = OSMT_PREPASS_ERR_FILL_ARENA;
        }
    }
    if (live) a.info[o] = oi;
}

__device__ __forceinline__ double opacity_by_center_distance(double cd, double hlw) {
    const double feather_from = fmax(hlw - 0.5, 0.0);
    const double feather_to = fmax(hlw + 0.5, 1.0);
    const double feather_dist = feather_to - feather_from;
    const double opacity_mul = fmin(2.0 * hlw, 1.0);
    double v;
    if (cd < feather_from)
        v = 1.0;
    else if (cd < feather_to)
        v = (feather_to - cd) / feather_dist;
    else
        v = 0.0;
    return opacity_mul * v;
}

#define OSMT_C4(i) (double)(i) / 255.0, (double)((i) + 1) / 255.0, (double)((i) + 2) / 255.0, (double)((i) + 3) / 255.0
#define OSMT_C16(i) OSMT_C4(i), OSMT_C4((i) + 4), OSMT_C4((i) + 8), OSMT_C4((i) + 12)
#define OSMT_C64(i) OSMT_C16(i), OSMT_C16((i) + 16), OSMT_C16((i) + 32), OSMT_C16((i) + 48)
__constant__ double k_u8_over_255[256] = {OSMT_C64(0), OSMT_C64(64), OSMT_C64(128), OSMT_C64(192)};

constexpr int SUB = OSMT_SUB_W;
constexpr int SUBH = OSMT_SUB_H;
constexpr int NTHREADS = 64;
constexpr int PXT = SUB * SUBH / NTHREADS;
constexpr int ROWSTEP = NTHREADS / SUB;
#ifndef OSMT_V_OPCHUNK
#define OSMT_V_OPCHUNK 16
#endif
constexpr int OPCHUNK = OSMT_V_OPCHUNK;
static_assert(OPCHUNK == 16 || OPCHUNK == 32 || OPCHUNK == 64, "a chunk is staged by one wave");
#ifndef OSMT_V_SEGCAP
#define OSMT_V_SEGCAP 32
#endif
constexpr int SEGCAP = OSMT_V_SEGCAP;
static_assert(SEGCAP >= 8 && SEGCAP <= 64, "a filter pass is at most one wave wide");
#ifndef OSMT_V_PLANE_STRIDE
#define OSMT_V_PLANE_STRIDE 32
#endif
constexpr int PLANE_STRIDE = OSMT_V_PLANE_STRIDE;

#if defined(OSMT_ABL) && OSMT_ABL == 5
#define OSMT_DBG(...) __VA_ARGS__
#else
#define OSMT_DBG(...)
#endif
struct alignas(16) StagedEnt {
    double c0, c1, c2;
    double op;
    uint32_t arena;
    uint32_t kind_stage;
    uint32_t aux;
    uint32_t nv;
};
static_assert(sizeof(StagedEnt) == 48, "three 16-byte LDS loads");
struct StrokeConst {
    double ff0, ft0, fd0, rfd0, mul0;
    uint32_t flags;
    uint32_t _pad;
};
constexpr uint32_t STROKE_PLAIN_MAIN = 1u;
constexpr uint32_t STROKE_UNIT_FD = 2u;
constexpr uint32_t STROKE_TINY_MUL = 4u;
constexpr uint32_t STROKE_DASH_FAST = 8u;
__device__ __forceinline__ uint32_t stroke_flags(const osmt_stroke_aux* __restrict__ sa) {
    const bool tiny = !(sa->mul0 >= 1e-100);
    const int n = sa->main_n_segs;
#ifdef OSMT_V_NO_DASH_FAST
    const bool fast = false;
#else
    const bool fast = n > 0 && sa->main_has_orig == 0 && sa->main_total_len > 0.0 && !tiny;
#endif
    return (n == 0 ? STROKE_PLAIN_MAIN : 0u) | (sa->fd0 == 1.0 ? STROKE_UNIT_FD : 0u) | (tiny ? STROKE_TINY_MUL : 0u) | (fast ? STROKE_DASH_FAST : 0u);
}
#ifndef OSMT_V_STAGECAP
#define OSMT_V_STAGECAP 16
#endif
constexpr int STAGECAP = OSMT_V_STAGECAP;

struct alignas(8) SegDer {
    int32_t a, b;
    float r2b, r2a;
    uint32_t w;
    uint32_t n_main;
    double ru, rv;
};
static_assert(sizeof(SegDer) == 40, "five 8-byte LDS words");
constexpr uint32_t SEGW_INCX_NEG = 1u, SEGW_INCY_NEG = 2u, SEGW_SWAP = 4u, SEGW_CAP = 8u, SEGW_SLOW = 16u;

#ifndef OSMT_V_FILTCAP
#define OSMT_V_FILTCAP 256
#endif
constexpr uint32_t FILTCAP = OSMT_V_FILTCAP;
#if OSMT_V_OPCHUNK <= OSMT_V_STAGECAP
#define OSMT_STAGE_UNION 1
#else
#define OSMT_STAGE_UNION 0
#endif
constexpr int DTAB_F = 7;
struct RasterShared {
    OSMT_DBG(uint32_t dbg[12];)
    osmt_srec seg[SEGCAP];
    SegDer der[SEGCAP];
    uint32_t pre[SEGCAP];
    unsigned long long plane[PLANE_STRIDE * SUBH];
    StagedEnt ent[OPCHUNK];
    uint32_t nvi[OPCHUNK];
#if OSMT_STAGE_UNION
    union {
        uint32_t fmask[SUBH];
        StrokeConst sconst;
    } stg[STAGECAP];
#else
    uint32_t fmask_[STAGECAP][SUBH];
    StrokeConst sconst_[STAGECAP];
#endif
    double dtab[OSMT_MAX_DASH_SEGS][DTAB_F];
    uint32_t queue[64];
#ifdef OSMT_V_LDSPAD
    uint8_t occupancy_experiment_pad[OSMT_V_LDSPAD];
#endif
};
#if !(defined(OSMT_ABL) && OSMT_ABL == 5)
static_assert(sizeof(RasterShared) <= 10240, "16 waves per CU (four per SIMD) share 160 KB of LDS");
#endif
#if OSMT_STAGE_UNION
#define SH_FMASK(sh, st) ((sh).stg[st].fmask)
#define SH_SCONST(sh, st) ((sh).stg[st].sconst)
#else
#define SH_FMASK(sh, st) ((sh).fmask_[st])
#define SH_SCONST(sh, st) ((sh).sconst_[st])
#endif
static_assert(FILTCAP <= sizeof(osmt_srec) * SEGCAP && 8u * SEGCAP <= sizeof(SegDer) * SEGCAP && FILTCAP % 256u == 0u,
              "the filter pass borrows seg[] for its entry marks (one 4-byte store per lane) and der[] for the kept slots");

struct SubRect {
    int32_t x0, y0, x1, y1;
};

__device__ __forceinline__ void blend_px(double* acc, double sr, double sg, double sb, double sa) {
    const double k = 1.0 - sa;
    acc[0] = sr + k * acc[0];
    acc[1] = sg + k * acc[1];
    acc[2] = sb + k * acc[2];
    acc[3] = sa + k * acc[3];
}
__device__ __forceinline__ void blend_rgb(double* acc, double sr, double sg, double sb, double sa) {
    const double k = 1.0 - sa;
    acc[0] = sr + k * acc[0];
// ... 334 lines not shown
                    if (dt > w_lo && dt < w_hi) {
                        if (kind == 1u) {
                            const double num = ft0 - cd;
                            const double qv = fd0 == 1.0 ? num : osmt_div_exact(num, fd0, rfd0);
                            const double cdop = mul0 * (cd < ff0 ? 1.0 : qv);
                            atomicMax(&sh.plane[st.ry * PLANE_STRIDE + st.rx], (unsigned long long)__double_as_longlong(initial_opacity * cdop));
                        }
                    } else {
                        slow = true;
                    }
                }
            }
            const unsigned long long sb = __ballot(slow);
            if (sb) {
                const uint32_t ns = (uint32_t)__popcll(sb);
                if (qn + ns > 64u) {
                    dashed_drain(sh, qn, kc, n, total, r_total, initial_opacity, rc);
                    qn = 0u;
                }
                if (slow) sh.queue[qn + (uint32_t)__popcll(sb & ((1ull << fresh_lane()) - 1ull))] = slot_tag | ((uint32_t)st.ry << 5) | (uint32_t)st.rx;
                qn += ns;
            }
            if (active) {
                const bool corr = st.err + st.two_a > st.b;
                dotv += corr ? dot_step + dot_corr : dot_step;
                walk_advance(st);
            }
        }
    }
    if (qn) dashed_drain(sh, qn, kc, n, total, r_total, initial_opacity, rc);
}

template <class Shared>
__device__ __forceinline__ void walk_items(Shared& sh, uint32_t lane, uint32_t slot0, uint32_t nslot, uint32_t item_base, uint32_t it_lo, uint32_t it_hi,
                                           const StrokeConst& kc, uint32_t sflags, const osmt_stroke_aux* __restrict__ sa, double initial_opacity,
                                           const SubRect& rc) {
    OSMT_DBG(if (lane == 0u) { sh.dbg[1] += (it_hi - it_lo + 63u) / 64u; sh.dbg[2] += it_hi - it_lo; })
    const bool main_plain = (sflags & STROKE_PLAIN_MAIN) != 0u;
    const bool unit_fd = (sflags & (STROKE_UNIT_FD | STROKE_TINY_MUL)) == STROKE_UNIT_FD;
    const bool dash_fast = (sflags & STROKE_DASH_FAST) != 0u;
    if (dash_fast) {
        walk_items_dashed(sh, slot0, nslot, item_base, it_lo, it_hi, kc, sa->main_n_segs, sa->main_total_len, sa->main_r_total, initial_opacity, rc);
        const uint32_t l_ = fresh_lane();
        if (!__ballot(l_ < nslot && (sh.der[slot0 + l_].w & SEGW_CAP) != 0u)) return;
    }
    for (uint32_t it = it_lo + lane; it < it_hi; it += 64u) {
        uint32_t lo_s = slot0, n = nslot;
        while (n > 1u) {
            const uint32_t half = n >> 1;
            const bool right = sh.pre[lo_s + half - 1u] <= it;
            lo_s = right ? lo_s + half : lo_s;
            n = right ? n - half : half;
        }
        const uint32_t base_items = (lo_s == slot0) ? item_base : sh.pre[lo_s - 1u];
        const osmt_srec& r = sh.seg[lo_s];
        const SegDer& d = sh.der[lo_s];
        const bool is_cap = (d.w & SEGW_CAP) != 0u;
        RunState st;
        bool skip_first;
        walk_setup(st, r, d, it - base_items, rc, &skip_first);
        if (main_plain && !is_cap) {
            if (unit_fd)
                walk_plain<true>(st, kc, initial_opacity, skip_first, sh.plane);
            else
                walk_plain<false>(st, kc, initial_opacity, skip_first, sh.plane);
        } else {
#ifndef OSMT_V_NODASH
#pragma unroll 1
            for (uint32_t t = main_plain ? 1u : 0u; t < 2u; ++t) {
                if (is_cap != (t == 1u)) continue;
                if (dash_fast && t == 0u) continue;
#ifdef OSMT_V_SKIPHEAVY
                if (t == (OSMT_V_SKIPHEAVY - 1)) continue;
#endif
                const bool cp = t == 1u;
                const osmt_raster_args* la = late_args();
                const osmt_dash_seg* sgs = cp ? &sa->caps_seg : la->dseg + (size_t)(sa - la->aux) * OSMT_MAX_DASH_SEGS;
                walk_dashed(st, kc, cp ? 1 : sa->main_n_segs, (cp ? sa->caps_has_orig : sa->main_has_orig) != 0, cp ? 0.0 : sa->main_total_len,
                            cp ? 0.0 : sa->main_r_total, sgs, sa->half_width, r.traveled, initial_opacity, sh.plane);
            }
#endif
        }
    }
}

__device__ __noinline__ uint32_t fill_row_streaming(const osmt_ring* __restrict__ rings, const int2* __restrict__ pts,
                                                    uint32_t ring_off, uint32_t n_rings, int32_t y, int32_t x0,
                                                    int32_t x1) {
    uint32_t m = 0u;
    int32_t last_x = INT32_MIN;
    int64_t last_e = -1;
    bool have_last = false;
    uint32_t k = 0;
    int32_t from_x = 0;
    for (;;) {
        bool found = false;
        int32_t bx = 0, bxm = 0;
        int64_t be = 0;
        uint32_t eb = 0;
        for (uint32_t r = 0; r < n_rings; ++r) {
            const osmt_ring ring = rings[ring_off + r];
            if (ring.n_pts < 2) continue;
            for (uint32_t e = 0; e + 1 < ring.n_pts; ++e) {
                const int2 p1 = pts[ring.first_pt + e];
                const int2 p2 = pts[ring.first_pt + e + 1];
                int32_t xmn, xmx;
                if (!osmt_fill_row_extent(p1.x, p1.y, p2.x, p2.y, y, &xmn, &xmx)) continue;
                const int64_t ge = (int64_t)eb + e;
                const bool after = !have_last || xmn > last_x || (xmn == last_x && ge > last_e);
                if (!after) continue;
                if (!found || xmn < bx || (xmn == bx && ge < be)) {
                    found = true;
                    bx = xmn;
                    bxm = xmx;
                    be = ge;
                }
            }
            eb += ring.n_pts - 1;
        }
        if (!found) break;
        if ((k & 1u) == 0u) {
            from_x = bx;
        } else {
            const int32_t from = max(from_x, x0);
            const int32_t to = min(bxm, x1);
            if (from <= to) {
                const uint32_t len = (uint32_t)(to - from + 1);
                const uint32_t bits = (len >= 32u) ? 0xFFFFFFFFu : ((1u << len) - 1u);
                m |= bits << (uint32_t)(from - x0);
            }
        }
        have_last = true;
        last_x = bx;
        last_e = be;
        ++k;
    }
    return m;
}

#ifndef OSMT_V_WAVES
#define OSMT_V_WAVES 4
#endif
#if OSMT_V_WAVES > 0
#define OSMT_RASTER_BOUNDS __launch_bounds__(NTHREADS) __attribute__((amdgpu_waves_per_eu(OSMT_V_WAVES, OSMT_V_WAVES)))
#else
#define OSMT_RASTER_BOUNDS __launch_bounds__(NTHREADS)
#endif
#ifdef OSMT_V_NORESTRICT
#define OSMT_R
#else
#define OSMT_R __restrict__
#endif

#ifndef OSMT_V_FILL_GROUP
#define OSMT_V_FILL_GROUP 2
#endif
constexpr uint32_t FILL_GROUP = OSMT_V_FILL_GROUP;
constexpr uint32_t FILL_EMAX = 128;
#ifndef OSMT_V_FILL_RMAX
#define OSMT_V_FILL_RMAX 384
#endif
constexpr uint32_t FILL_RMAX = OSMT_V_FILL_RMAX;
struct FillShared {
    int32_t r_xmin[FILL_RMAX];
    int32_t r_xmax[FILL_RMAX];
    uint32_t r_key[FILL_RMAX];
    int2 e_p1[FILL_EMAX], e_p2[FILL_EMAX];
    int32_t e_y0[FILL_EMAX];
    uint32_t e_lane0[FILL_EMAX];
    uint32_t e_pre[FILL_EMAX];
    uint32_t e_key[FILL_EMAX];
    int32_t diff[65];
    uint32_t rowfill[64];
    uint32_t rowstart[64];
};

__device__ __forceinline__ void fill_rows_body(FillShared& sh, const uint32_t group, const uint32_t lane, const osmt_op* __restrict__ g_ops,
                                               uint32_t n_ops, const osmt_opinfo* __restrict__ g_info, const osmt_ring* __restrict__ g_rings,
                                               const int2* __restrict__ g_pts, const uint32_t* __restrict__ g_op_blk,
                                               const osmt_blk_bbox* __restrict__ g_blk, uint32_t scale, uint32_t sub_rows,
                                               uint32_t* __restrict__ g_submask, uint32_t* __restrict__ g_fmask,
                                               const uint32_t* __restrict__ g_op_job, uint32_t* __restrict__ g_cnt) {
    const uint32_t o_first = group * FILL_GROUP;
    const uint32_t n_sub_x = OSMT_TILE_SIZE * scale / SUB;
    uint32_t g_geom[FILL_GROUP], g_arena[FILL_GROUP], g_base[FILL_GROUP + 1];
    uint32_t g_ne[FILL_GROUP], g_pt0[FILL_GROUP];
    g_base[0] = 0u;
#pragma unroll
    for (uint32_t k = 0; k < FILL_GROUP; ++k) {
        uint32_t geom = 0u, arena = 0u, ne = 0u, pt0 = 0u;
        if (o_first + k < n_ops) {
            const osmt_opinfo* __restrict__ oi = &g_info[o_first + k];
            const uint32_t kind = oi->kind;
            if (kind == OSMT_OP_FILL_COLOR || kind == OSMT_OP_FILL_IMAGE) {
                geom = oi->fill_geom;
                arena = oi->arena_off;
                ne = 0xFFFFFFFFu;
                if (oi->n_rings == 1u && oi->n_edges <= 16u) {
                    ne = oi->n_edges;
                    pt0 = oi->first_pt;
                }
            }
        }
        g_geom[k] = (uint32_t)__builtin_amdgcn_readfirstlane((int)geom);
        g_arena[k] = (uint32_t)__builtin_amdgcn_readfirstlane((int)arena);
        g_ne[k] = (uint32_t)__builtin_amdgcn_readfirstlane((int)ne);
        g_pt0[k] = (uint32_t)__builtin_amdgcn_readfirstlane((int)pt0);
        g_base[k + 1] = g_base[k] + (g_geom[k] >> 24);
    }
    const uint32_t n_slots = g_base[FILL_GROUP];
    if (n_slots == 0u) return;
    sh.rowfill[lane] = 0u;
    sh.diff[lane] = 0;
    if (lane == 0u) sh.diff[64] = 0;
    __syncthreads();
    for (uint32_t t0 = 0; t0 < n_slots; t0 += 4u) {
        const uint32_t t = t0 + (lane >> OSMT_SUB_H_LOG2);
        const bool row_valid = t < n_slots;
        uint32_t my_k = 0u;
#pragma unroll
        for (uint32_t k = 1; k < FILL_GROUP; ++k)
            if (t >= g_base[k] && g_base[k] < n_slots) my_k = k;
        uint32_t geom = g_geom[0], arena = g_arena[0], base = g_base[0];
#pragma unroll
        for (uint32_t k = 1; k < FILL_GROUP; ++k)
            if (my_k == k) {
                geom = g_geom[k];
                arena = g_arena[k];
                base = g_base[k];
            }
        const uint32_t my_o = o_first + my_k;
        const uint32_t sr0 = geom & 255u, c0 = (geom >> 8) & 255u, ncols = row_valid ? (geom >> 16) & 255u : 0u;
        const uint32_t sr = sr0 + (t - base);
        const int32_t y = (int32_t)(sr * SUBH + (lane & (SUBH - 1u)));
        uint32_t row_hit = 0u;

        uint32_t w0 = 0u, ww = 64u;
        while (w0 < 64u) {
            const bool in_win = lane >= w0 && lane < w0 + ww;
            uint32_t n_list = 0u, n_cross = 0u;
            bool overflow = false;
            bool pooled = true;
#pragma unroll
            for (uint32_t k = 0; k < FILL_GROUP; ++k) {
                const uint32_t s_lo = max(g_base[k], t0), s_hi = min(g_base[k + 1], t0 + 4u);
                if (s_lo < s_hi && max((s_lo - t0) * SUBH, w0) < min((s_hi - t0) * SUBH, w0 + ww) && g_ne[k] == 0xFFFFFFFFu) pooled = false;
            }
            if (pooled) {
                uint32_t kq[4] = {0xFFu, 0xFFu, 0xFFu, 0xFFu}, nq = 0u;
#pragma unroll
                for (uint32_t q = 0; q < FILL_GROUP; ++q)
                    if (max(g_base[q], t0) < min(g_base[q + 1], t0 + 4u)) {
                        if (nq == 0u) kq[0] = q;
                        if (nq == 1u) kq[1] = q;
                        if (nq == 2u) kq[2] = q;
                        if (nq == 3u) kq[3] = q;
                        ++nq;
                    }
                const uint32_t qi = lane >> 4, e = lane & 15u;
                const uint32_t k = qi == 0u ? kq[0] : (qi == 1u ? kq[1] : (qi == 2u ? kq[2] : kq[3]));
                uint32_t kbase = g_base[0], kend = k == 0u ? g_base[1] : 0u, kgeom = g_geom[0], kne = k == 0u ? g_ne[0] : 0u, kpt0 = g_pt0[0];
#pragma unroll
                for (uint32_t q = 1; q < FILL_GROUP; ++q)
                    if (k == q) {
                        kbase = g_base[q];
                        kend = g_base[q + 1];
                        kgeom = g_geom[q];
                        kne = g_ne[q];
                        kpt0 = g_pt0[q];
                    }
                const uint32_t s_lo = max(kbase, t0), s_hi = min(kend, t0 + 4u);
                uint32_t cnt = 0u, l0 = 0u;
                int32_t first = 0;
                int2 p1 = make_int2(0, 0), p2 = p1;
                if (s_lo < s_hi && e < kne) {
                    const uint32_t la = max((s_lo - t0) * SUBH, w0), lb = min((s_hi - t0) * SUBH, w0 + ww);
                    if (la < lb) {
                        const int32_t ybase = ((int32_t)(kgeom & 255u) + (int32_t)t0 - (int32_t)kbase) * SUBH;
                        const int32_t ya = ybase + (int32_t)la, yb = ybase + (int32_t)lb - 1;
                        p1 = g_pts[kpt0 + e];
                        p2 = g_pts[kpt0 + e + 1u];
                        const int32_t ytop = min(p1.y, p2.y), ybot = max(p1.y, p2.y);
                        first = max(ytop + 1, ya);
                        const int32_t last = min(ybot, yb);
                        cnt = last >= first ? (uint32_t)(last - first + 1) : 0u;
                        l0 = la + (uint32_t)(first - ya);
                    }
                }
                const unsigned long long has = __ballot(cnt != 0u);
                if (has != 0ull) {
                    const uint32_t incl = wave_incl_scan(cnt);
                    const uint32_t pos = (uint32_t)__popcll(has & ((1ull << lane) - 1ull));
                    n_list = (uint32_t)__popcll(has);
                    n_cross = (uint32_t)__builtin_amdgcn_readlane((int)incl, 63);
                    if (n_cross > FILL_RMAX) {
                        overflow = true;
                    } else if (cnt != 0u) {
                        sh.e_p1[pos] = p1;
                        sh.e_p2[pos] = p2;
                        sh.e_y0[pos] = first;
                        sh.e_lane0[pos] = l0;
                        sh.e_pre[pos] = incl;
                        sh.e_key[pos] = e;
                        atomicAdd(&sh.diff[l0], 1);
                        atomicAdd(&sh.diff[l0 + cnt], -1);
                    }
                }
            } else
#pragma unroll 1
            for (uint32_t k = 0; k < FILL_GROUP; ++k) {
                const uint32_t s_lo = max(g_base[k], t0), s_hi = min(g_base[k + 1], t0 + 4u);
                if (s_lo >= s_hi) continue;
                const uint32_t la = max((s_lo - t0) * SUBH, w0), lb = min((s_hi - t0) * SUBH, w0 + ww);
                if (la >= lb) continue;
                const uint32_t o = o_first + k;
                const int32_t ybase = ((int32_t)(g_geom[k] & 255u) + (int32_t)t0 - (int32_t)g_base[k]) * SUBH;
                const int32_t ya = ybase + (int32_t)la, yb = ybase + (int32_t)lb - 1;
                const osmt_op* __restrict__ op = &g_ops[o];
                const uint32_t ring_off = op->ring_off, n_rings = op->n_rings;
                const uint32_t blk_off = g_op_blk[o];
                uint32_t ring_cur = 0u, e_base = 0u;
                for (uint32_t R0 = 0; ring_cur < n_rings; R0 += 64u) {
                    const uint32_t E = R0 + lane;
                    uint32_t pt = 0xFFFFFFFFu;
                    while (ring_cur < n_rings) {
                        const osmt_ring ring = g_rings[ring_off + ring_cur];
                        const uint32_t ne = ring.n_pts >= 2u ? ring.n_pts - 1u : 0u;
                        if (E >= e_base && E < e_base + ne) pt = ring.first_pt + (E - e_base);
                        if (e_base + ne > R0 + 64u) break;
                        e_base += ne;
                        ++ring_cur;
                    }
                    if (blk_off != 0xFFFFFFFFu) {
                        const osmt_blk_bbox bb = g_blk[blk_off + (R0 >> 6)];
                        if (bb.y1 < ya || bb.y0 >= yb) continue;
                    }
                    uint32_t cnt = 0u;
                    int32_t first = 0;
                    int2 p1 = make_int2(0, 0), p2 = p1;
                    if (pt != 0xFFFFFFFFu) {
                        p1 = g_pts[pt];
                        p2 = g_pts[pt + 1u];
                        const int32_t ytop = min(p1.y, p2.y), ybot = max(p1.y, p2.y);
                        first = max(ytop + 1, ya);
                        const int32_t last = min(ybot, yb);
                        cnt = last >= first ? (uint32_t)(last - first + 1) : 0u;
                    }
                    const unsigned long long has = __ballot(cnt != 0u);
                    if (has == 0ull) continue;
                    const uint32_t incl = wave_incl_scan(cnt);
                    const uint32_t pos = n_list + (uint32_t)__popcll(has & ((1ull << lane) - 1ull));
                    n_list += (uint32_t)__popcll(has);
                    const uint32_t n_before = n_cross;
                    n_cross += (uint32_t)__builtin_amdgcn_readlane((int)incl, 63);
                    if (n_list > FILL_EMAX || n_cross > FILL_RMAX) {
                        overflow = true;
                        continue;
                    }
                    if (cnt != 0u && !overflow) {
                        sh.e_p1[pos] = p1;
                        sh.e_p2[pos] = p2;
                        sh.e_y0[pos] = first;
                        const uint32_t l0 = la + (uint32_t)(first - ya);
                        sh.e_lane0[pos] = l0;
                        sh.e_pre[pos] = n_before + incl;
                        sh.e_key[pos] = E;
                        atomicAdd(&sh.diff[l0], 1);
                        atomicAdd(&sh.diff[l0 + cnt], -1);
                    }
                }
            }
            __syncthreads();
            const int32_t d = sh.diff[lane];
            sh.diff[lane] = 0;
            if (lane == 0u) sh.diff[64] = 0;
            if (overflow) {
                __syncthreads();
                if (ww > 1u) {
                    ww >>= 1;
                    continue;
                }
                if (in_win && row_valid) {
                    const osmt_op* __restrict__ op = &g_ops[my_o];
                    for (uint32_t c = 0; c < ncols; ++c) {
                        const int32_t x0 = (int32_t)((c0 + c) * SUB);
                        const uint32_t m = fill_row_streaming(g_rings, g_pts, op->ring_off, op->n_rings, y, x0, x0 + SUB - 1);
                        g_fmask[((size_t)arena + (size_t)(sr - sr0) * ncols + c) * SUBH + (lane & (SUBH - 1u))] = m;
                        if (m) row_hit |= 1u << (c0 + c);
                    }
                }
            }
            if (!overflow) {
                const uint32_t rc_incl = wave_incl_scan((uint32_t)d);
                const uint32_t rowcnt = in_win ? rc_incl : 0u;
                const uint32_t rowstart = wave_incl_scan(rowcnt) - rowcnt;
                sh.rowstart[lane] = rowstart;
                __syncthreads();
#if defined(OSMT_ABL) && OSMT_ABL == 11
                if (false)
#endif
                for (uint32_t i = lane; i < n_cross; i += 64u) {
                    uint32_t lo = 0u, n = n_list;
                    while (n > 1u) {
                        const uint32_t half = n >> 1;
                        const bool right = sh.e_pre[lo + half - 1u] <= i;
                        lo = right ? lo + half : lo;
                        n = right ? n - half : half;
                    }
                    const uint32_t kk = i - (lo ? sh.e_pre[lo - 1u] : 0u);
                    const int2 p1 = sh.e_p1[lo], p2 = sh.e_p2[lo];
                    const uint32_t L = sh.e_lane0[lo] + kk;
                    int32_t xmn = 0, xmx = 0;
                    osmt_fill_row_extent(p1.x, p1.y, p2.x, p2.y, sh.e_y0[lo] + (int32_t)kk, &xmn, &xmx);
                    const uint32_t at = sh.rowstart[L] + atomicAdd(&sh.rowfill[L], 1u);
                    sh.r_xmin[at] = xmn;
                    sh.r_xmax[at] = xmx;
                    sh.r_key[at] = sh.e_key[lo];
                }
                __syncthreads();
                sh.rowfill[lane] = 0u;
#if defined(OSMT_ABL) && (OSMT_ABL == 11 || OSMT_ABL == 12)
                if (false) {
#else
                if (in_win && row_valid) {
#endif
                    for (uint32_t i = 1; i < rowcnt; ++i) {
                        const int32_t kx = sh.r_xmin[rowstart + i], km = sh.r_xmax[rowstart + i];
                        const uint32_t ke = sh.r_key[rowstart + i];
                        int32_t j = (int32_t)i - 1;
                        while (j >= 0) {
                            const int32_t jx = sh.r_xmin[rowstart + (uint32_t)j];
                            const uint32_t je = sh.r_key[rowstart + (uint32_t)j];
                            if (!(jx > kx || (jx == kx && je > ke))) break;
                            sh.r_xmin[rowstart + (uint32_t)j + 1u] = jx;
                            sh.r_xmax[rowstart + (uint32_t)j + 1u] = sh.r_xmax[rowstart + (uint32_t)j];
                            sh.r_key[rowstart + (uint32_t)j + 1u] = je;
                            --j;
                        }
                        sh.r_xmin[rowstart + (uint32_t)(j + 1)] = kx;
                        sh.r_xmax[rowstart + (uint32_t)(j + 1)] = km;
                        sh.r_key[rowstart + (uint32_t)(j + 1)] = ke;
                    }
                    for (uint32_t c = 0; c < ncols; ++c) {
                        const int32_t x0 = (int32_t)((c0 + c) * SUB), x1 = x0 + SUB - 1;
                        uint32_t m = 0u;
                        for (uint32_t k2 = 0; k2 + 1u < rowcnt; k2 += 2u) {
                            const int32_t from = max(sh.r_xmin[rowstart + k2], x0);
                            const int32_t to = min(sh.r_xmax[rowstart + k2 + 1u], x1);
                            if (from <= to) {
                                const uint32_t len = (uint32_t)(to - from + 1);
                                const uint32_t bits = (len >= 32u) ? 0xFFFFFFFFu : ((1u << len) - 1u);
                                m |= bits << (uint32_t)(from - x0);
                            }
                        }
                        g_fmask[((size_t)arena + (size_t)(sr - sr0) * ncols + c) * SUBH + (lane & (SUBH - 1u))] = m;
                        if (m) row_hit |= 1u << (c0 + c);
                    }
                }
                __syncthreads();
            }
            w0 += ww;
            while (ww < 64u && (w0 & (2u * ww - 1u)) == 0u) ww <<= 1;
        }
        uint32_t hm = row_hit;
        hm |= (uint32_t)__builtin_amdgcn_update_dpp(0, (int)hm, 0x111, 0xF, 0xF, false);
        hm |= (uint32_t)__builtin_amdgcn_update_dpp(0, (int)hm, 0x112, 0xF, 0xF, false);
        hm |= (uint32_t)__builtin_amdgcn_update_dpp(0, (int)hm, 0x114, 0xF, 0xF, false);
        hm |= (uint32_t)__builtin_amdgcn_update_dpp(0, (int)hm, 0x118, 0xF, 0xF, false);
        if (row_valid && (lane & (SUBH - 1u)) == SUBH - 1u) {
            g_submask[(size_t)my_o * sub_rows + sr] = hm;
            uint32_t* ct = g_cnt + ((size_t)g_op_job[my_o] * sub_rows + sr) * n_sub_x;
            while (hm) {
                atomicAdd(ct + (uint32_t)__builtin_ctz(hm), 1u);
                hm &= hm - 1u;
            }
        }
    }
}

struct StrokeBinSeg {
    osmt_srec rec;
    double ft;
    int32_t sx0, sy0;
    uint32_t ncols;
    uint32_t slot0;
    uint32_t op, job;
    uint32_t is_cap;
    uint32_t _pad;
};
struct StrokeBinShared {
    uint32_t incl[OSMT_BIN_SEGS];
    StrokeBinSeg seg[OSMT_BIN_SEGS];
};

__device__ __forceinline__ void stroke_bin_body(StrokeBinShared& sh, const uint32_t blk, const uint32_t lane,
                                                const osmt_opinfo* __restrict__ g_info, uint32_t n_vsegs,
                                                uint32_t scale, uint32_t sub_rows, uint32_t* __restrict__ g_submask,
                                                osmt_srec* __restrict__ g_srec, uint2* __restrict__ g_skey, const uint32_t* __restrict__ g_op_job,
                                                uint32_t* __restrict__ g_cnt, const osmt_vseg* __restrict__ g_vseg) {
    const uint32_t g = blk * OSMT_BIN_SEGS + lane;
    const int32_t W = (int32_t)(OSMT_TILE_SIZE * scale);
    const int32_t n_sub_x = W / SUB, n_sub_y = (int32_t)sub_rows;
    uint32_t n_pairs = 0u;
    if (lane < OSMT_BIN_SEGS && g < n_vsegs) {
        const osmt_vseg vsr = g_vseg[g];
        const uint32_t vo = vsr.vop;
        const int4 pp = make_int4(vsr.p1x, vsr.p1y, vsr.p2x, vsr.p2y);
        const uint32_t o = vo & 0x7FFFFFFFu;
        StrokeBinSeg sg;
        sg.is_cap = vo >> 31;
        sg.rec.p1x = pp.x; sg.rec.p1y = pp.y; sg.rec.p2x = pp.z; sg.rec.p2y = pp.w;
        sg.rec.traveled = vsr.trav;
        sg.rec.denom = vsr.den;
        sg.rec.rdenom = vsr.rden;
        const uint32_t cand_off = vsr.cand_off;
        if (!(sg.rec.p1x == sg.rec.p2x && sg.rec.p1y == sg.rec.p2y)) {
            const osmt_opinfo* __restrict__ oi = &g_info[o];
            sg.ft = oi->stroke_ft;
            const uint32_t rec_cap = oi->rec_cap, arena_off = oi->arena_off;
            const SubWindow w = vseg_window(sg.rec.p1x, sg.rec.p1y, sg.rec.p2x, sg.rec.p2y, sg.rec.denom, sg.ft, n_sub_x, n_sub_y);
            const uint32_t wc = window_count(w);
            if (wc && (unsigned long long)cand_off + wc <= rec_cap) {
                sg.sx0 = w.sx0;
                sg.sy0 = w.sy0;
                sg.ncols = (uint32_t)(w.sx1 - w.sx0 + 1);
                sg.slot0 = arena_off + cand_off;
                sg.op = o;
                sg.job = g_op_job[o];
                sg._pad = 0u;
                sg.rec.k_lo0 = sg.rec.k_lo1 = sg.rec.m_lo0 = sg.rec.m_lo1 = 0;
                sg.rec.k_n0 = sg.rec.k_n1 = sg.rec.n_x0 = sg.rec.n_x1 = 0;
                sh.seg[lane] = sg;
                n_pairs = wc;
            }
        }
    }
    const uint32_t incl = wave_incl_scan(n_pairs);
    if (lane < OSMT_BIN_SEGS) sh.incl[lane] = incl;
    const uint32_t total = (uint32_t)__builtin_amdgcn_readlane((int)incl, 63);
    __syncthreads();
    for (uint32_t i = lane; i < total; i += 64u) {
        uint32_t v = 0u;
#pragma unroll
        for (uint32_t step = OSMT_BIN_SEGS / 2u; step; step >>= 1)
            if (sh.incl[v + step - 1u] <= i) v += step;
        const StrokeBinSeg& sg = sh.seg[v];
        const uint32_t j = i - (v ? sh.incl[v - 1u] : 0u);
        const uint32_t ncols = sg.ncols;
        uint32_t qy = (uint32_t)((float)j * __builtin_amdgcn_rcpf((float)ncols));
        if ((qy + 1u) * ncols <= j) ++qy;
        if (qy * ncols > j) --qy;
        const int32_t sx = sg.sx0 + (int32_t)(j - qy * ncols), sy = sg.sy0 + (int32_t)qy;
        const int32_t x0 = sx * SUB, y0 = sy * SUBH;
        osmt_srec rec = sg.rec;
        osmt_item_ranges ir;
        const uint32_t cnt = osmt_seg_ranges(rec.p1x, rec.p1y, rec.p2x, rec.p2y, rec.denom, sg.ft, x0, y0, x0 + SUB - 1, y0 + SUBH - 1, &ir);
        const size_t slot = (size_t)sg.slot0 + j;
        if (cnt == 0u) {
            g_skey[slot] = make_uint2(0xFFFFFFFFu, 0u);
            continue;
        }
        rec.k_lo0 = ir.k_lo0; rec.k_n0 = (uint16_t)ir.k_n0; rec.k_lo1 = ir.k_lo1; rec.k_n1 = (uint16_t)ir.k_n1;
        rec.m_lo0 = ir.m_lo0; rec.n_x0 = (uint16_t)ir.n_x0; rec.m_lo1 = ir.m_lo1; rec.n_x1 = (uint16_t)ir.n_x1;
        g_srec[slot] = rec;
        g_skey[slot] = make_uint2((uint32_t)(sy * n_sub_x + sx), cnt | (sg.is_cap << 31));
        const uint32_t bit = 1u << sx;
        if (!(atomicOr(&g_submask[(size_t)sg.op * sub_rows + (uint32_t)sy], bit) & bit))
            atomicAdd(g_cnt + ((size_t)sg.job * sub_rows + (uint32_t)sy) * (uint32_t)n_sub_x + (uint32_t)sx, 1u);
    }
}

__global__ __launch_bounds__(64) void k_prebin(const osmt_op* __restrict__ g_ops, uint32_t n_ops, const osmt_opinfo* __restrict__ g_info,
                                               const osmt_ring* __restrict__ g_rings, const int2* __restrict__ g_pts,
                                               const uint32_t* __restrict__ g_op_blk,
                                               const osmt_blk_bbox* __restrict__ g_blk, uint32_t n_vsegs, const osmt_prebin_map roles,
                                               uint32_t scale, uint32_t sub_rows, uint32_t* __restrict__ g_submask,
                                               uint32_t* __restrict__ g_fmask,
                                               osmt_srec* __restrict__ g_srec, uint2* __restrict__ g_skey, const uint32_t* __restrict__ g_op_job,
                                               uint32_t* __restrict__ g_cnt, const osmt_vseg* __restrict__ g_vseg) {
    __shared__ union {
        FillShared fill;
        StrokeBinShared bin;
    } shu;
    uint32_t idx;
    const bool stroke = osmt_prebin_role(roles, blockIdx.x, &idx) != 0u;
#if defined(OSMT_ABL) && OSMT_ABL == 9
    if (stroke) return;
#endif
#if defined(OSMT_ABL) && OSMT_ABL == 10
    if (!stroke) return;
#endif
    if (stroke)
        stroke_bin_body(shu.bin, idx, threadIdx.x, g_info, n_vsegs, scale, sub_rows, g_submask,
                        g_srec, g_skey, g_op_job, g_cnt, g_vseg);
    else
        fill_rows_body(shu.fill, idx, threadIdx.x, g_ops, n_ops, g_info, g_rings, g_pts, g_op_blk, g_blk, scale, sub_rows, g_submask, g_fmask,
                       g_op_job, g_cnt);
}

#ifndef OSMT_V_SUBLIST_THREADS
#define OSMT_V_SUBLIST_THREADS 1024
#endif
constexpr uint32_t SUBLIST_THREADS = OSMT_V_SUBLIST_THREADS;
#ifndef OSMT_V_SUBLIST_AHEAD
#define OSMT_V_SUBLIST_AHEAD 4
#endif
constexpr uint32_t SUBLIST_AHEAD = OSMT_V_SUBLIST_AHEAD;
constexpr uint32_t SUBLIST_MAX_SUB = (OSMT_TILE_SIZE * OSMT_MAX_SCALE / OSMT_SUB_W) * (OSMT_TILE_SIZE * OSMT_MAX_SCALE / OSMT_SUB_H);
__global__ __launch_bounds__(SUBLIST_THREADS) void k_sublist(const osmt_tile_job* __restrict__ g_jobs, uint32_t g_scale,
                                                             const osmt_opinfo* __restrict__ g_info, const uint32_t* __restrict__ g_submask,
                                                             uint32_t g_sub_rows, const uint32_t* __restrict__ g_cnt,
                                                             unsigned long long* __restrict__ g_cursor, unsigned long long* __restrict__ g_lcur,
                                                             uint2* __restrict__ g_hdr,
                                                             osmt_ent* __restrict__ g_ent, unsigned long long ent_cap, uint32_t* g_err,
                                                             uint32_t g_fold_max_ops) {
    __shared__ uint32_t s_off[SUBLIST_MAX_SUB];
    __shared__ uint32_t s_base[2];
    __shared__ uint2 s_q[SUBLIST_THREADS / 64u][128];
    const uint32_t tid = threadIdx.x, lane = tid & 63u, wave = tid >> 6;
    const uint32_t tile = blockIdx.x;
    if (g_fold_max_ops != 0u && g_jobs[tile].n_ops <= g_fold_max_ops) return;
    const uint32_t W = OSMT_TILE_SIZE * g_scale;
    const uint32_t nsx = W / SUB;
    const uint32_t nsub = nsx * g_sub_rows;
    const uint32_t* __restrict__ cnt = g_cnt + (size_t)tile * nsub;
    const osmt_tile_job job = g_jobs[tile];
    const uint32_t n_ops = job.n_ops;
    for (uint32_t i = tid; i < nsub; i += SUBLIST_THREADS) s_off[i] = cnt[i];
    auto load_bits = [&](uint32_t sy, uint32_t b0) -> uint32_t {
        const uint32_t i = b0 + lane;
        return (i < n_ops && sy < g_sub_rows) ? g_submask[(size_t)(job.op_off + i) * g_sub_rows + sy] : 0u;
    };
    struct OpRaw {
        uint32_t aux;
        uint4 a, b;
    };
    static_assert(offsetof(osmt_opinfo, aux) == 16 && offsetof(osmt_opinfo, kind) == 32 && offsetof(osmt_opinfo, color) == 34 &&
                      offsetof(osmt_opinfo, arena_off) == 40 && offsetof(osmt_opinfo, rec_cap) == 44 &&
                      offsetof(osmt_opinfo, fill_geom) == 48 && offsetof(osmt_opinfo, image_id) == 52 && offsetof(osmt_opinfo, opacity) == 56,
                  "k_sublist reads osmt_opinfo as three vector loads");
    struct OpRec {
        osmt_ent e;
        uint32_t geom, arena0;
        bool is_stroke;
    };
    auto fetch = [&](uint32_t w, uint32_t op) -> OpRaw {
        OpRaw r;
        r.aux = 0u;
        r.a = make_uint4(0u, 0u, 0u, 0u);
        r.b = make_uint4(0u, 0u, 0u, 0u);
        if (w != 0u) {
            const char* __restrict__ hi = reinterpret_cast<const char*>(&g_info[job.op_off + op]);
            r.aux = *reinterpret_cast<const uint32_t*>(hi + 16);
            r.a = *reinterpret_cast<const uint4*>(hi + 32);
            r.b = *reinterpret_cast<const uint4*>(hi + 48);
        }
        return r;
    };
    auto unpack = [&](const OpRaw& q) -> OpRec {
        OpRec r;
        r.e = {};
        const uint32_t kind = q.a.x & 255u;
        r.is_stroke = kind == OSMT_OP_STROKE;
        r.arena0 = q.a.z;
        r.geom = q.b.x;
        r.e.kind_color = kind | ((q.a.x >> 16) << 8) | (q.a.y << 24);
        r.e.opacity = __hiloint2double((int)q.b.w, (int)q.b.z);
        r.e.aux = r.is_stroke ? q.aux : q.b.y;
        r.e.nv = r.is_stroke ? q.a.w : 0u;
        return r;
    };
    const uint32_t pre_w = load_bits(wave, 0u);
    __syncthreads();
    if (wave == 0u) {
        const uint32_t per = (nsub + 63u) / 64u;
        const uint32_t i0 = min(lane * per, nsub), i1 = min(i0 + per, nsub);
        uint32_t sum = 0;
        for (uint32_t i = i0; i < i1; ++i) sum += s_off[i];
        const uint32_t incl = wave_incl_scan(sum);
        uint32_t run = incl - sum;
        for (uint32_t i = i0; i < i1; ++i) {
            const uint32_t c = s_off[i];
            s_off[i] = run;
            run += c;
        }
        const uint32_t total = (uint32_t)__builtin_amdgcn_readlane((int)incl, 63);
        if (lane == 0u) {
            const osmt_list_layout lay = osmt_list_layout_make(gridDim.x, ent_cap);
            const uint32_t slice = osmt_list_slice_of(lay, tile);
            unsigned long long* const cur = lay.n_slices > 1u ? g_lcur + (size_t)slice * OSMT_LIST_CURSOR_STRIDE : g_cursor;
            unsigned long long first = 0ull;
            uint32_t ok = 1u;
            if (total) {
                ok = osmt_list_place(lay, slice, atomicAdd(cur, (unsigned long long)total), total, &first);
                if (!ok && lay.n_slices > 1u)
                    ok = osmt_list_place_overflow(lay, ent_cap, atomicAdd(g_lcur + (size_t)lay.n_slices * OSMT_LIST_CURSOR_STRIDE, (unsigned long long)total),
                                                  total, &first);
            }
            s_base[0] = (uint32_t)first;
            s_base[1] = ok;
            if (!s_base[1] && g_err) *(volatile uint32_t*)g_err = OSMT_PREPASS_ERR_LIST_ARENA;
        }
    }
    __syncthreads();
    const uint32_t base = s_base[0];
    const bool fits = s_base[1] != 0u;
    const unsigned long long lanes_below = (1ull << lane) - 1ull;
    for (uint32_t sy = wave; sy < g_sub_rows; sy += SUBLIST_THREADS / 64u) {
        uint32_t cur = 0u, row_n = 0u;
        if (lane < nsx) {
            const uint32_t c = cnt[sy * nsx + lane];
            cur = base + s_off[sy * nsx + lane];
            row_n = fits ? c : 0u;
            g_hdr[(size_t)tile * nsub + sy * nsx + lane] = make_uint2(cur, row_n);
        }
        if (__ballot(row_n != 0u) == 0ull) continue;
        const bool first_row = sy == wave;
        auto work = [&](const uint32_t w, const OpRaw& raw) {
            const OpRec rec = unpack(raw);
            osmt_ent e = rec.e;
            const uint32_t geom = rec.geom, arena0 = rec.arena0;
            const bool is_stroke = rec.is_stroke;
            const uint32_t sr0 = geom & 255u, c0 = (geom >> 8) & 255u, ncols = (geom >> 16) & 255u;
            for (uint32_t sx = 0; sx < nsx; ++sx) {
                const bool hit = (w >> sx) & 1u;
                const unsigned long long bal = __ballot(hit);
                if (bal == 0ull) continue;
                const uint32_t col_cur = (uint32_t)__builtin_amdgcn_readlane((int)cur, (int)sx);
                const uint32_t col_left = (uint32_t)__builtin_amdgcn_readlane((int)row_n, (int)sx);
                const uint32_t pos = (uint32_t)__popcll(bal & lanes_below);
                if (hit && pos < col_left) {
                    e.arena = is_stroke ? arena0 : (arena0 + (sy - sr0) * ncols + (sx - c0)) * SUBH;
                    g_ent[(size_t)col_cur + pos] = e;
                }
                const uint32_t took = min((uint32_t)__popcll(bal), col_left);
                if (lane == sx) {
                    cur += took;
                    row_n -= took;
                }
            }
        };
        constexpr uint32_t PD = SUBLIST_AHEAD;
        uint2* const q = s_q[wave];
        uint32_t head = 0u, tail = 0u;
        bool have = false;
        uint32_t w_p = 0u;
        OpRaw raw_p = {};
        auto request = [&](uint32_t n) {
            __builtin_amdgcn_wave_barrier();
            asm volatile("" ::: "memory");
// ... 659 lines not shown
            __builtin_nontemporal_store(v, out);
#endif
            OSMT_DBG(__syncthreads(); if (j == 0 && ly_o == 0 && lx_o < 12) *out = sh.dbg[lx_o];)
        }
    }
}

typedef double v2d __attribute__((ext_vector_type(2)));

__device__ __forceinline__ double dpp_swap_pair(double x) {
    const long long b = __double_as_longlong(x);
    const int lo = __builtin_amdgcn_update_dpp(0, (int)(b & 0xFFFFFFFFll), 0xB1, 0xF, 0xF, false);
    const int hi = __builtin_amdgcn_update_dpp(0, (int)(b >> 32), 0xB1, 0xF, 0xF, false);
    return __longlong_as_double(((long long)hi << 32) | (unsigned int)lo);
}

template <int LT, bool NT>
__global__ __launch_bounds__(256) void k_composite(const v2d* __restrict__ planes, double4 canvas, uint32_t n,
                                                   uint32_t L, uint32_t npx, uint32_t* __restrict__ out) {
    const size_t total_runs = (size_t)n * (npx / 64u);
    const uint32_t lane = threadIdx.x & 63u;
    const size_t wave0 = ((size_t)blockIdx.x * 256u + threadIdx.x) >> 6;
    const size_t nwaves = ((size_t)gridDim.x * 256u) >> 6;
    const bool odd = lane & 1u;
    for (size_t run = wave0; run < total_runs; run += nwaves) {
        const size_t t = run / (npx / 64u);
        const size_t q0 = (run - t * (npx / 64u)) * 64u;
        const v2d* src = planes + ((t * (size_t)L) * npx + q0) * 2u + lane;
        const size_t layer_stride = (size_t)npx * 2u;
        double d[4] = {canvas.x, canvas.y, canvas.z, canvas.w};
        auto blend_layer = [&](v2d h0, v2d h1) {
            const v2d give = odd ? h0 : h1;
            v2d got;
            got.x = dpp_swap_pair(give.x);
            got.y = dpp_swap_pair(give.y);
            const v2d rg = odd ? got : h0;
            const v2d ba = odd ? h1 : got;
            blend_px(d, rg.x, rg.y, ba.x, ba.y);
        };
        if (LT > 0) {
            v2d h0[LT > 0 ? LT : 1], h1[LT > 0 ? LT : 1];
#pragma unroll
            for (int l = 0; l < LT; ++l) {
                if (NT) {
                    h0[l] = __builtin_nontemporal_load(src + (size_t)l * layer_stride);
                    h1[l] = __builtin_nontemporal_load(src + (size_t)l * layer_stride + 64);
                } else {
                    h0[l] = src[(size_t)l * layer_stride];
                    h1[l] = src[(size_t)l * layer_stride + 64];
                }
            }
#pragma unroll
            for (int l = 0; l < LT; ++l) blend_layer(h0[l], h1[l]);
        } else {
            for (uint32_t l = 0; l < L; ++l) {
                const v2d a0 = __builtin_nontemporal_load(src + (size_t)l * layer_stride);
                const v2d a1 = __builtin_nontemporal_load(src + (size_t)l * layer_stride + 64);
                blend_layer(a0, a1);
            }
        }
        const double a = d[3];
        const double mr = (a == 0.0) ? 0.0 : d[0] / a;
        const double mg = (a == 0.0) ? 0.0 : d[1] / a;
        const double mb = (a == 0.0) ? 0.0 : d[2] / a;
        const size_t px = t * npx + q0 + (lane >> 1) + (odd ? 32u : 0u);
        out[px] = f64_as_u8(255.0 * mr) | (f64_as_u8(255.0 * mg) << 8) | (f64_as_u8(255.0 * mb) << 16) | 0xFF000000u;
    }
}

typedef uint32_t v4u __attribute__((ext_vector_type(4)));
__global__ __launch_bounds__(256) void k_copy16(const v4u* __restrict__ src, v4u* __restrict__ dst, size_t n) {
    const size_t stride = (size_t)gridDim.x * 1024u;
    size_t i = (size_t)blockIdx.x * 1024u + threadIdx.x;
    for (; i + 768u < n; i += stride) {
        const v4u a = __builtin_nontemporal_load(src + i), b = __builtin_nontemporal_load(src + i + 256u);
        const v4u c = __builtin_nontemporal_load(src + i + 512u), d = __builtin_nontemporal_load(src + i + 768u);
        __builtin_nontemporal_store(a, dst + i);
        __builtin_nontemporal_store(b, dst + i + 256u);
        __builtin_nontemporal_store(c, dst + i + 512u);
        __builtin_nontemporal_store(d, dst + i + 768u);
    }
    for (uint32_t k = 0; k < 4u; ++k)
        if (i + 256u * k < n && i + 768u >= n) __builtin_nontemporal_store(__builtin_nontemporal_load(src + i + 256u * k), dst + i + 256u * k);
}
__global__ __launch_bounds__(256) void k_read16(const v4u* __restrict__ src, uint32_t* __restrict__ sink, size_t n) {
    const size_t stride = (size_t)gridDim.x * 1024u;
    v4u acc = {0u, 0u, 0u, 0u};
    size_t i = (size_t)blockIdx.x * 1024u + threadIdx.x;
    for (; i + 768u < n; i += stride) {
        const v4u a = __builtin_nontemporal_load(src + i), b = __builtin_nontemporal_load(src + i + 256u);
        const v4u c = __builtin_nontemporal_load(src + i + 512u), d = __builtin_nontemporal_load(src + i + 768u);
        acc ^= a ^ b ^ c ^ d;
    }
    for (uint32_t k = 0; k < 4u; ++k)
        if (i + 256u * k < n && i + 768u >= n) acc ^= __builtin_nontemporal_load(src + i + 256u * k);
    const uint32_t w = acc.x ^ acc.y ^ acc.z ^ acc.w;
    if (w == 0x9E3779B9u) sink[blockIdx.x] = w;
}

}

hipError_t osmt_launch_copy16(const void* src, void* dst, size_t n16, bool read_only, hipStream_t st) {
    if (n16 == 0) return hipSuccess;
    const size_t blocks = (n16 + 1023) / 1024;
    const uint32_t grid = (uint32_t)(blocks < 256 * 16 ? blocks : 256 * 16);
    if (read_only)
        hipLaunchKernelGGL(k_read16, dim3(grid), dim3(256), 0, st, reinterpret_cast<const v4u*>(src), reinterpret_cast<uint32_t*>(dst), n16);
    else
        hipLaunchKernelGGL(k_copy16, dim3(grid), dim3(256), 0, st, reinterpret_cast<const v4u*>(src), reinterpret_cast<v4u*>(dst), n16);
    return hipGetLastError();
}

hipError_t osmt_launch_project(const osmt_tile_job* jobs, const uint32_t* pt_job, const double* latlon, const uint32_t* refs,
                               uint32_t n_pts, double scale, int32_t* pts, hipStream_t st, uint32_t* zero, size_t n_zero) {
    const size_t n_thr = n_pts > n_zero ? n_pts : n_zero;
    if (n_thr == 0) return hipSuccess;
    hipLaunchKernelGGL(k_project, dim3((uint32_t)((n_thr + 255u) / 256u)), dim3(256), 0, st, jobs, pt_job,
                       reinterpret_cast<const double2*>(latlon), refs, n_pts, scale, reinterpret_cast<int2*>(pts), zero, (uint32_t)n_zero);
    return hipGetLastError();
}

size_t osmt_prepass_zero_words(const osmt_prepass_args& a) {
    const uint32_t Wt = OSMT_TILE_SIZE * a.scale;
    const size_t n_cnt = (a.fmask_cap || a.srec_cap) ? (size_t)a.n_jobs * (Wt / SUB) * (Wt / SUBH) : 0;
    if (n_cnt && osmt_list_layout_make(a.n_jobs, a.ent_cap).n_slices > 1u) return osmt_list_cursor_word0(n_cnt) + OSMT_LIST_CURSOR_WORDS;
    return 4 * sizeof(unsigned long long) / sizeof(uint32_t) + n_cnt;
}

hipError_t osmt_launch_ptjob(const osmt_tile_job* jobs, uint32_t n_jobs, uint32_t* pt_job, uint32_t n_pts, hipStream_t st) {
    if (n_pts == 0) return hipSuccess;
    hipError_t e = hipMemsetAsync(pt_job, 0xFF, (size_t)n_pts * 4, st);
    if (e != hipSuccess) return e;
    if (n_jobs) hipLaunchKernelGGL(k_ptjob, dim3(n_jobs), dim3(256), 0, st, jobs, pt_job);
    return hipGetLastError();
}

hipError_t osmt_launch_project_single(const double* latlon, uint32_t n, uint32_t zoom, uint32_t tx, uint32_t ty,
                                      double scale, int32_t* pts, hipStream_t st) {
    if (n == 0) return hipSuccess;
    hipLaunchKernelGGL(k_project_single, dim3((n + 255u) / 256u), dim3(256), 0, st,
                       reinterpret_cast<const double2*>(latlon), n, zoom, tx, ty, scale, reinterpret_cast<int2*>(pts));
    return hipGetLastError();
}

hipError_t osmt_launch_prepass(const osmt_prepass_args& a, hipStream_t st, bool zeroed) {
    if (!zeroed) {
        const hipError_t e = hipMemsetAsync(a.cursors, 0, osmt_prepass_zero_words(a) * sizeof(uint32_t), st);
        if (e != hipSuccess) return e;
    }
    if (a.n_ops)
        hipLaunchKernelGGL(k_opinfo, dim3((a.n_ops + OPINFO_THREADS * OPINFO_WAVES - 1u) / (OPINFO_THREADS * OPINFO_WAVES)),
                           dim3(OPINFO_THREADS * OPINFO_WAVES), 0, st, a);
    if (a.fmask_cap == 0 && a.srec_cap == 0) return hipGetLastError();
    const osmt_prebin_map roles = osmt_prebin_map_make(osmt_prebin_n_vblk(a.n_vsegs, OSMT_BIN_SEGS), (a.n_ops + FILL_GROUP - 1u) / FILL_GROUP);
    if (a.n_ops)
        hipLaunchKernelGGL(k_prebin, dim3(roles.n_vblk + roles.n_fgrp), dim3(64), 0, st, a.ops, a.n_ops, a.info, a.rings, a.pts,
                           a.op_blk, a.blk, a.n_vsegs, roles,
                           a.scale, a.sub_rows, a.submask, a.fmask, a.srec, a.skey, a.op_job, a.cnt, a.vseg);
    if (a.n_jobs && (a.fold_max_ops == 0u || a.max_job_ops > a.fold_max_ops)) {
        const uint32_t Wt = OSMT_TILE_SIZE * a.scale;
        unsigned long long* const lcur = reinterpret_cast<unsigned long long*>(
            reinterpret_cast<uint32_t*>(a.cursors) + osmt_list_cursor_word0((size_t)a.n_jobs * (Wt / SUB) * (Wt / SUBH)));
        hipLaunchKernelGGL(k_sublist, dim3(a.n_jobs), dim3(SUBLIST_THREADS), 0, st, a.jobs, a.scale, a.info, a.submask, a.sub_rows, a.cnt,
                           a.cursors + 2, lcur, a.hdr, a.ent, a.ent_cap, a.err, a.fold_max_ops);
    }
    return hipGetLastError();
}

hipError_t osmt_launch_raster(const osmt_raster_args& a, bool out_f64, hipStream_t st) {
    if (a.n_jobs == 0) return hipSuccess;
    const uint32_t W = OSMT_TILE_SIZE * a.scale;
    const uint32_t nsub = (W / SUB) * (W / SUBH);
    const uint32_t groups = (a.n_jobs + 7u) / 8u;
    const dim3 grid(groups * 8u * nsub);
#define OSMT_LAUNCH_RASTER(F64, LAB)                                                                \
    do {                                                                                            \
        if (a.fold_max_ops)                                                                         \
            hipLaunchKernelGGL((k_raster<F64, LAB, true>), grid, dim3(NTHREADS), 0, st, a);  \
        else                                                                                        \
            hipLaunchKernelGGL((k_raster<F64, LAB, false>), grid, dim3(NTHREADS), 0, st, a); \
    } while (0)
    if (out_f64)
        OSMT_LAUNCH_RASTER(true, false);
    else if (a.labels.info)
        OSMT_LAUNCH_RASTER(false, true);
    else
        OSMT_LAUNCH_RASTER(false, false);
#undef OSMT_LAUNCH_RASTER
    return hipGetLastError();
}

#ifndef OSMT_V_COMP_NT
#define OSMT_V_COMP_NT 1
#endif
#ifndef OSMT_V_COMP_BLOCKS
#define OSMT_V_COMP_BLOCKS 16
#endif
hipError_t osmt_launch_composite(const void* planes, const double canvas[4], uint32_t n, uint32_t L, uint32_t npx,
                                 void* out, hipStream_t st) {
    const size_t total = (size_t)n * npx;
    if (total == 0) return hipSuccess;
    if (npx % 64u) return hipErrorInvalidValue;
    const double4 cv = make_double4(canvas[0], canvas[1], canvas[2], canvas[3]);
    size_t blocks = (total + 255) / 256;
    const size_t cap = 256 * OSMT_V_COMP_BLOCKS;
    if (blocks > cap) blocks = cap;
    const v2d* p = reinterpret_cast<const v2d*>(planes);
    uint32_t* o = reinterpret_cast<uint32_t*>(out);
    constexpr bool NT = OSMT_V_COMP_NT != 0;
    if (L == 8)
        hipLaunchKernelGGL((k_composite<8, NT>), dim3((uint32_t)blocks), dim3(256), 0, st, p, cv, n, L, npx, o);
    else if (L == 4)
        hipLaunchKernelGGL((k_composite<4, NT>), dim3((uint32_t)blocks), dim3(256), 0, st, p, cv, n, L, npx, o);
    else
        hipLaunchKernelGGL((k_composite<0, NT>), dim3((uint32_t)blocks), dim3(256), 0, st, p, cv, n, L, npx, o);
    return hipGetLastError();
}
```

osm_renderer_amd/csrc/osmt_prebin_roles.h:

```cpp
#ifndef OSMT_PREBIN_ROLES_H
#define OSMT_PREBIN_ROLES_H

#include <stdint.h>

#if !defined(OSMT_HD)
#if defined(__HIPCC__)
#define OSMT_HD __host__ __device__ __forceinline__
#else
#define OSMT_HD inline
#endif
#endif

#ifndef OSMT_V_BIN_SEGS
#define OSMT_V_BIN_SEGS 32
#endif
#if OSMT_V_BIN_SEGS != 64 && OSMT_V_BIN_SEGS != 32 && OSMT_V_BIN_SEGS != 16
#error "OSMT_V_BIN_SEGS is 64, 32 or 16"
#endif
#define OSMT_BIN_SEGS ((uint32_t)OSMT_V_BIN_SEGS)

#ifndef OSMT_V_PREBIN_INTERLEAVE
#define OSMT_V_PREBIN_INTERLEAVE 1
#endif

struct osmt_prebin_map {
    uint32_t n_vblk, n_fgrp;
    uint64_t magic;
};

OSMT_HD uint32_t osmt_prebin_n_vblk(uint32_t n_vsegs, uint32_t bin_segs) {
    return n_vsegs / bin_segs + (n_vsegs % bin_segs ? 1u : 0u);
}

OSMT_HD osmt_prebin_map osmt_prebin_map_make(uint32_t n_vblk, uint32_t n_fgrp) {
    osmt_prebin_map m;
    m.n_vblk = n_vblk;
    m.n_fgrp = n_fgrp;
    const uint64_t T = (uint64_t)n_vblk + n_fgrp;
    m.magic = T ? ~(uint64_t)0 / T : 0u;
    return m;
}

OSMT_HD uint64_t osmt_mulhi64(uint64_t a, uint64_t b) {
#if defined(__HIP_DEVICE_COMPILE__)
    return __umul64hi(a, b);
#else
    return (uint64_t)(((unsigned __int128)a * b) >> 64);
#endif
}

OSMT_HD uint32_t osmt_prebin_role(const osmt_prebin_map m, uint32_t b, uint32_t* idx) {
#if OSMT_V_PREBIN_INTERLEAVE
    const uint64_t T = (uint64_t)m.n_vblk + m.n_fgrp;
    const uint64_t x = (uint64_t)b * m.n_vblk;
    uint64_t s = osmt_mulhi64(x, m.magic);
    uint64_t r = x - s * T;
    if (r >= T) {
        r -= T;
        ++s;
    }
    if (r + m.n_vblk >= T) {
        *idx = (uint32_t)s;
        return 1u;
    }
    *idx = b - (uint32_t)s;
    return 0u;
#else
    if (b < m.n_vblk) {
        *idx = b;
        return 1u;
    }
    *idx = b - m.n_vblk;
    return 0u;
#endif
}

#endif
```

Measured before the change: 1.464 million tiles/s.

## Compact fill sub-rows into a dense slot queue for prebin fill blocks

k_opinfo now reserves per-workgroup slot ranges with an atomic cursor and writes one compact slot record per fill sub-row (op, fmask offset, geometry, simple-ring edge info), padded to multiples of four. The prebin fill role reads four slots per pass instead of rescanning op groups with variable sub-row counts. This removes idle blocks for non-fill ops and the per-group selection logic, so each wave works on full slots. The cost is an extra arena buffer, extra atomics and padding writes in opinfo, and a grid size sized from a host-side count that is measured only on the sizing path.

```diff
diff --git a/osm_renderer_amd/build.py b/osm_renderer_amd/build.py
--- a/osm_renderer_amd/build.py
+++ b/osm_renderer_amd/build.py
@@ -6,7 +6,7 @@
 CSRC = os.path.join(HERE, "csrc")
 LIB = os.path.join(HERE, "libosmtile.so")
 SOURCES = ["osmt_kernels.hip", "osmt_labels.hip", "osmt_glyphs.hip", "osmt_textplace.hip", "osmt_textshape.hip", "osmt_polylabel.hip", "osmt_styled.hip", "osmt_tilequery.hip", "osmt_tilelabels.hip", "osmt_arealabels.hip", "osmt_selmatch.hip", "osmt_labelbind.hip", "osmt_cascade.hip", "osmt_anchors.hip", "osmt_pngenc.hip", "osmt_api.cpp", "osmt_png.cpp"]
-HEADERS = ["osmt_bitonic.h", "osmt_cascade_rule.h", "osmt_cascade_tables.h", "osmt_geom.h", "osmt_glyph.h", "osmt_internal.h", "osmt_list_slices.h", "osmt_numparse.h", "osmt_png_table.h", "osmt_prebin_roles.h", "osmt_project.h", "osmt_utf8.h", os.path.join("..", "host", "osmt_textplacer.hpp"),
+HEADERS = ["osmt_bitonic.h", "osmt_cascade_rule.h", "osmt_cascade_tables.h", "osmt_fill_slots.h", "osmt_geom.h", "osmt_glyph.h", "osmt_internal.h", "osmt_list_slices.h", "osmt_numparse.h", "osmt_png_table.h", "osmt_prebin_roles.h", "osmt_project.h", "osmt_utf8.h", os.path.join("..", "host", "osmt_textplacer.hpp"),
            os.path.join("..", "host", "osmt_textshaper.hpp"),
            os.path.join("..", "..", "include", "osmtile.h")]
 LIBS = ["-lz", "-ldl", "-lpthread", "-Wl,--no-undefined"]
diff --git a/osm_renderer_amd/csrc/osmt_api.cpp b/osm_renderer_amd/csrc/osmt_api.cpp
--- a/osm_renderer_amd/csrc/osmt_api.cpp
+++ b/osm_renderer_amd/csrc/osmt_api.cpp
@@ -231,6 +231,9 @@
     osmt_srec* d_srec = nullptr;
     uint2* d_skey = nullptr;
     unsigned long long fmask_cap = 0, srec_cap = 0;
+    osmt_fill_slot* d_slots = nullptr;
+    unsigned long long slot_cap = 0;
+    uint32_t n_fill_pass = 0;
     std::vector<uint32_t> h_pt_job, h_op_aux, h_op_blk, h_op_vseg, h_op_job, h_lab_wide;
     std::vector<osmt_label_band> h_lab_bands;
     std::vector<osmt_labelinfo> h_lab_info;
@@ -884,6 +887,9 @@
     a.skey = sc->d_skey;
     a.fmask_cap = sizing ? 0ull : sc->fmask_cap;
     a.srec_cap = sizing ? 0ull : sc->srec_cap;
+    a.slots = sc->d_slots;
+    a.slot_cap = sizing ? 0ull : sc->slot_cap;
+    a.n_fill_pass = sc->n_fill_pass;
     a.err = sizing ? nullptr : sc->h_err;
     return a;
 }
@@ -1128,11 +1134,12 @@
             HIP_TRY(osmt_launch_project(s->d_jobs, s->d_pt_job, s->d_latlon, s->coord_kind == OSMT_COORD_NODE_REF ? s->d_node_refs : nullptr,
                                         s->n_pts, (double)s->scale, s->d_pts, st));
         HIP_TRY(osmt_launch_prepass(prepass_args(s, true), st));
-        unsigned long long totals[2] = {0ull, 0ull};
+        unsigned long long totals[4] = {0ull, 0ull, 0ull, 0ull};
         HIP_TRY(hipMemcpyAsync(totals, s->d_cursors, sizeof totals, hipMemcpyDeviceToHost, st));
         HIP_TRY(hipStreamSynchronize(st));
         groups = totals[0];
         recs = totals[1];
+        s->n_fill_pass = (uint32_t)std::max<unsigned long long>(std::min<unsigned long long>(totals[3] / OSMT_FILL_PASS_SLOTS, 0x7FFFFFFFull), 1ull);
         std::lock_guard<std::mutex> lk(ctx->cache_mu);
         osmt_ctx::arena_density& d = ctx->density[s->scale];
         if (n_fills) d.groups_per_fill = std::max(d.groups_per_fill * 0.98, (double)groups / (double)n_fills);
@@ -1159,6 +1166,8 @@
     const size_t o_k = carve((size_t)(recs + 1) * 8);
     const osmt_list_layout lay = osmt_list_layout_make(s->n_jobs, ents + 1);
     const size_t o_e = carve((size_t)lay.total * sizeof(osmt_ent));
+    const unsigned long long slot_cap = osmt_fill_slot_capacity(groups, n_fills, (uint32_t)(W / OSMT_SUB_H), s->n_ops);
+    const size_t o_q = carve((size_t)slot_cap * sizeof(osmt_fill_slot));
     hipError_t e = dev_alloc(ctx, (void**)&s->d_arena, off + 256);
     if (e != hipSuccess) {
         s->d_arena = nullptr;
@@ -1169,6 +1178,8 @@
     s->d_skey = (uint2*)(s->d_arena + o_k);
     s->d_ent = (osmt_ent*)(s->d_arena + o_e);
     s->ent_cap = ents + 1;
+    s->d_slots = (osmt_fill_slot*)(s->d_arena + o_q);
+    s->slot_cap = slot_cap;
     static const bool trace_arenas = getenv("OSMT_TRACE_UPLOAD") != nullptr;
     if (trace_arenas)
         fprintf(stderr, "osmt arenas: %u tiles, fill groups %llu, stroke records %llu, list entries %llu in %u slice(s) of %llu (+ overflow): "
diff --git a/osm_renderer_amd/csrc/osmt_fill_slots.h b/osm_renderer_amd/csrc/osmt_fill_slots.h
--- /dev/null
+++ b/osm_renderer_amd/csrc/osmt_fill_slots.h
@@ -0,0 +1,75 @@
+#ifndef OSMT_FILL_SLOTS_H
+#define OSMT_FILL_SLOTS_H
+
+#include <stdint.h>
+
+#if !defined(OSMT_HD)
+#if defined(__HIPCC__)
+#define OSMT_HD __host__ __device__ __forceinline__
+#else
+#define OSMT_HD inline
+#endif
+#endif
+
+#define OSMT_FILL_PASS_SLOTS 4u
+#ifndef OSMT_V_OPINFO_THREADS
+#define OSMT_V_OPINFO_THREADS 64
+#endif
+#ifndef OSMT_V_OPINFO_WAVES
+#define OSMT_V_OPINFO_WAVES 8
+#endif
+#define OSMT_FILL_SLOT_WG_OPS ((uint32_t)(OSMT_V_OPINFO_THREADS * OSMT_V_OPINFO_WAVES))
+
+struct alignas(16) osmt_fill_slot {
+    uint32_t op;
+    uint32_t word0;
+    uint32_t geom;
+    uint32_t first_pt;
+};
+#define OSMT_FILL_SLOT_SIMPLE 0x80000000u
+#define OSMT_FILL_SLOT_MAX_SIMPLE_EDGES 16u
+
+OSMT_HD osmt_fill_slot osmt_fill_slot_empty(void) {
+    osmt_fill_slot s;
+    s.op = 0xFFFFFFFFu;
+    s.word0 = 0u;
+    s.geom = 0u;
+    s.first_pt = 0u;
+    return s;
+}
+
+OSMT_HD osmt_fill_slot osmt_fill_slot_make(uint32_t op, uint32_t arena_off, uint32_t r, uint32_t sr0, uint32_t c0, uint32_t ncols,
+                                           uint32_t n_rings, uint32_t n_edges, uint32_t first_pt) {
+    osmt_fill_slot s;
+    s.op = op;
+    s.word0 = (arena_off + r * ncols) * 16u;
+    s.geom = (sr0 + r) | (c0 << 8) | (ncols << 16);
+    if (n_rings == 1u && n_edges <= OSMT_FILL_SLOT_MAX_SIMPLE_EDGES) s.geom |= (n_edges << 24) | OSMT_FILL_SLOT_SIMPLE;
+    s.first_pt = first_pt;
+    return s;
+}
+OSMT_HD uint32_t osmt_fill_slot_sr(uint32_t geom) { return geom & 255u; }
+OSMT_HD uint32_t osmt_fill_slot_c0(uint32_t geom) { return (geom >> 8) & 255u; }
+OSMT_HD uint32_t osmt_fill_slot_ncols(uint32_t geom) { return (geom >> 16) & 255u; }
+OSMT_HD uint32_t osmt_fill_slot_simple(uint32_t geom) { return geom >> 31; }
+OSMT_HD uint32_t osmt_fill_slot_edges(uint32_t geom) { return (geom >> 24) & 31u; }
+
+OSMT_HD uint32_t osmt_fill_slots_round(uint32_t total) { return (total + OSMT_FILL_PASS_SLOTS - 1u) & ~(OSMT_FILL_PASS_SLOTS - 1u); }
+
+OSMT_HD uint32_t osmt_fill_slot_first(uint32_t before_wave, uint32_t incl_in_wave, uint32_t nsr) { return before_wave + (incl_in_wave - nsr); }
+
+OSMT_HD uint32_t osmt_fill_slot_wgs(uint32_t n_ops) { return n_ops / OSMT_FILL_SLOT_WG_OPS + (n_ops % OSMT_FILL_SLOT_WG_OPS ? 1u : 0u); }
+
+OSMT_HD uint64_t osmt_fill_slot_capacity(uint64_t groups, uint64_t n_fills, uint32_t sub_rows, uint32_t n_ops) {
+    const uint64_t by_ops = n_fills * sub_rows;
+    const uint64_t real = groups < by_ops ? groups : by_ops;
+    const uint64_t cap = real + (uint64_t)(OSMT_FILL_PASS_SLOTS - 1u) * osmt_fill_slot_wgs(n_ops);
+    return (cap + OSMT_FILL_PASS_SLOTS - 1u) & ~(uint64_t)(OSMT_FILL_PASS_SLOTS - 1u);
+}
+
+OSMT_HD uint32_t osmt_fill_pass_count(uint64_t cursor, uint64_t capacity) {
+    const uint64_t n = cursor < capacity ? cursor : capacity;
+    return (uint32_t)(n / OSMT_FILL_PASS_SLOTS);
+}
+
+#endif
diff --git a/osm_renderer_amd/csrc/osmt_internal.h b/osm_renderer_amd/csrc/osmt_internal.h
--- a/osm_renderer_amd/csrc/osmt_internal.h
+++ b/osm_renderer_amd/csrc/osmt_internal.h
@@ -7,6 +7,7 @@
 #include "../../include/osmtile.h"
 #include "osmt_glyph.h"
 #include "osmt_list_slices.h"
+#include "osmt_fill_slots.h"
 
 #define OSMT_SUB_W 32
 #ifndef OSMT_SUB_H_LOG2
@@ -240,6 +241,9 @@
     uint32_t* submask;
     osmt_vseg* vseg;
     unsigned long long* cursors;
+    osmt_fill_slot* slots;
+    unsigned long long slot_cap;
+    uint32_t n_fill_pass;
     uint32_t* cnt;
     uint2* hdr;
     osmt_ent* ent;
diff --git a/osm_renderer_amd/csrc/osmt_kernels.hip b/osm_renderer_amd/csrc/osmt_kernels.hip
--- a/osm_renderer_amd/csrc/osmt_kernels.hip
+++ b/osm_renderer_amd/csrc/osmt_kernels.hip
@@ -135,15 +135,10 @@
     return (uint32_t)(w.sx1 - w.sx0 + 1) * (uint32_t)(w.sy1 - w.sy0 + 1);
 }
 
-#ifndef OSMT_V_OPINFO_THREADS
-#define OSMT_V_OPINFO_THREADS 64
-#endif
 constexpr uint32_t OPINFO_THREADS = OSMT_V_OPINFO_THREADS;
 static_assert(OPINFO_THREADS == 64 || OPINFO_THREADS == 32 || OPINFO_THREADS == 16, "the wave scans read their totals from the last active lane");
-#ifndef OSMT_V_OPINFO_WAVES
-#define OSMT_V_OPINFO_WAVES 8
-#endif
 constexpr uint32_t OPINFO_WAVES = OSMT_V_OPINFO_WAVES;
+static_assert(OPINFO_THREADS * OPINFO_WAVES == OSMT_FILL_SLOT_WG_OPS, "one slot reservation per workgroup");
 static_assert(OPINFO_WAVES == 1 || OPINFO_THREADS == 64, "several waves per workgroup: whole waves");
 __global__ __launch_bounds__(OPINFO_THREADS * OPINFO_WAVES) void k_opinfo(const osmt_prepass_args a) {
     const uint32_t op_lane = threadIdx.x % OPINFO_THREADS, op_wave = threadIdx.x / OPINFO_THREADS;
@@ -334,6 +329,10 @@
         const uint32_t f = (uint32_t)want_f;
         const uint32_t s_lo = (uint32_t)want_s & 0xFFFFu, s_hi = (uint32_t)(want_s >> 16);
         const uint32_t f_incl = wave_incl_scan(f);
+        const uint32_t nsr = want_f ? fill_geom_ok >> 24 : 0u;
+        const uint32_t q_incl = wave_incl_scan(nsr);
+        const uint32_t q_tot = (uint32_t)__builtin_amdgcn_readlane((int)q_incl, OPINFO_THREADS - 1);
+        uint32_t q_base = 0u;
         const unsigned long long s_incl = ((unsigned long long)wave_incl_scan(s_hi) << 16) + wave_incl_scan(s_lo);
         const uint32_t f_tot = (uint32_t)__builtin_amdgcn_readlane((int)f_incl, OPINFO_THREADS - 1);
         const unsigned long long s_tot = ((unsigned long long)(uint32_t)__builtin_amdgcn_readlane((int)(uint32_t)(s_incl >> 32), OPINFO_THREADS - 1) << 32) |
@@ -343,12 +342,20 @@
             if (lane == 0u) {
                 if (f_tot) f_base = atomicAdd(&a.cursors[0], (unsigned long long)f_tot);
                 if (s_tot) s_base = atomicAdd(&a.cursors[1], s_tot);
+                if (q_tot) {
+                    const uint32_t q_res = osmt_fill_slots_round(q_tot);
+                    q_base = (uint32_t)atomicAdd(&a.cursors[3], (unsigned long long)q_res);
+                    for (uint32_t i = q_tot; i < q_res; ++i)
+                        if ((unsigned long long)q_base + i < a.slot_cap) a.slots[q_base + i] = osmt_fill_slot_empty();
+                }
             }
         } else {
             __shared__ unsigned long long s_tot_f[OPINFO_WAVES], s_tot_s[OPINFO_WAVES];
+            __shared__ uint32_t s_tot_q[OPINFO_WAVES];
             if (lane == 0u) {
                 s_tot_f[op_wave] = f_tot;
                 s_tot_s[op_wave] = s_tot;
+                s_tot_q[op_wave] = q_tot;
             }
             __syncthreads();
             if (threadIdx.x == 0u) {
@@ -366,11 +373,26 @@
                     bf += tf;
                     bs += ts;
                 }
+                uint32_t bq = 0u;
+                for (uint32_t w = 0; w < OPINFO_WAVES; ++w) bq += s_tot_q[w];
+                if (bq) {
+                    const uint32_t q_res = osmt_fill_slots_round(bq);
+                    const uint32_t q0 = (uint32_t)atomicAdd(&a.cursors[3], (unsigned long long)q_res);
+                    for (uint32_t i = bq; i < q_res; ++i)
+                        if ((unsigned long long)q0 + i < a.slot_cap) a.slots[q0 + i] = osmt_fill_slot_empty();
+                    bq = q0;
+                }
+                for (uint32_t w = 0; w < OPINFO_WAVES; ++w) {
+                    const uint32_t tq = s_tot_q[w];
+                    s_tot_q[w] = bq;
+                    bq += tq;
+                }
             }
             __syncthreads();
             if (lane == 0u) {
                 f_base = s_tot_f[op_wave];
                 s_base = s_tot_s[op_wave];
+                q_base = s_tot_q[op_wave];
             }
         }
         f_base = ((unsigned long long)(uint32_t)__builtin_amdgcn_readfirstlane((int)(uint32_t)(f_base >> 32)) << 32) |
@@ -392,6 +414,22 @@
                 oi.fill_geom = fill_geom_ok;
             else if (a.err)
                 *(volatile uint32_t*)a.err = OSMT_PREPASS_ERR_FILL_ARENA;
+        }
+        q_base = (uint32_t)__builtin_amdgcn_readfirstlane((int)q_base);
+        if (nsr && a.slot_cap) {
+            const uint32_t first = q_base + osmt_fill_slot_first(0u, q_incl, nsr);
+            const uint32_t g = oi.fill_geom;
+            bool past = false;
+            for (uint32_t r = 0; r < nsr; ++r) {
+                if ((unsigned long long)first + r >= a.slot_cap) {
+                    past = true;
+                    break;
+                }
+                a.slots[first + r] = g ? osmt_fill_slot_make(o, oi.arena_off, r, g & 255u, (g >> 8) & 255u, (g >> 16) & 255u, oi.n_rings,
+                                                             oi.n_edges, oi.first_pt)
+                                       : osmt_fill_slot_empty();
+            }
+            if (past && a.err) *(volatile uint32_t*)a.err = OSMT_PREPASS_ERR_FILL_ARENA;
         }
     }
     if (live) a.info[o] = oi;
@@ -1032,10 +1070,11 @@
 #define OSMT_R __restrict__
 #endif
 
-#ifndef OSMT_V_FILL_GROUP
-#define OSMT_V_FILL_GROUP 2
-#endif
-constexpr uint32_t FILL_GROUP = OSMT_V_FILL_GROUP;
+#ifndef OSMT_V_FILL_BLOCK_PASSES
+#define OSMT_V_FILL_BLOCK_PASSES 2
+#endif
+constexpr uint32_t FILL_BLOCK_PASSES = OSMT_V_FILL_BLOCK_PASSES;
+static_assert(FILL_BLOCK_PASSES >= 1u, "a fill block runs at least one pass");
 constexpr uint32_t FILL_EMAX = 128;
 #ifndef OSMT_V_FILL_RMAX
 #define OSMT_V_FILL_RMAX 384
@@ -1055,65 +1094,35 @@
     uint32_t rowstart[64];
 };
 
-__device__ __forceinline__ void fill_rows_body(FillShared& sh, const uint32_t group, const uint32_t lane, const osmt_op* __restrict__ g_ops,
-                                               uint32_t n_ops, const osmt_opinfo* __restrict__ g_info, const osmt_ring* __restrict__ g_rings,
+__device__ __forceinline__ uint32_t fill_sel4(const uint32_t (&v)[4], uint32_t k) { return k == 0u ? v[0] : (k == 1u ? v[1] : (k == 2u ? v[2] : v[3])); }
+
+__device__ __forceinline__ void fill_rows_body(FillShared& sh, const uint32_t fblk, const uint32_t n_fblk, const uint32_t n_pass, const uint32_t lane,
+                                               const osmt_op* __restrict__ g_ops, const osmt_fill_slot* __restrict__ g_slots,
+                                               const osmt_ring* __restrict__ g_rings,
                                                const int2* __restrict__ g_pts, const uint32_t* __restrict__ g_op_blk,
                                                const osmt_blk_bbox* __restrict__ g_blk, uint32_t scale, uint32_t sub_rows,
                                                uint32_t* __restrict__ g_submask, uint32_t* __restrict__ g_fmask,
                                                const uint32_t* __restrict__ g_op_job, uint32_t* __restrict__ g_cnt) {
-    const uint32_t o_first = group * FILL_GROUP;
     const uint32_t n_sub_x = OSMT_TILE_SIZE * scale / SUB;
-    uint32_t g_geom[FILL_GROUP], g_arena[FILL_GROUP], g_base[FILL_GROUP + 1];
-    uint32_t g_ne[FILL_GROUP], g_pt0[FILL_GROUP];
-    g_base[0] = 0u;
-#pragma unroll
-    for (uint32_t k = 0; k < FILL_GROUP; ++k) {
-        uint32_t geom = 0u, arena = 0u, ne = 0u, pt0 = 0u;
-        if (o_first + k < n_ops) {
-            const osmt_opinfo* __restrict__ oi = &g_info[o_first + k];
-            const uint32_t kind = oi->kind;
-            if (kind == OSMT_OP_FILL_COLOR || kind == OSMT_OP_FILL_IMAGE) {
-                geom = oi->fill_geom;
-                arena = oi->arena_off;
-                ne = 0xFFFFFFFFu;
-                if (oi->n_rings == 1u && oi->n_edges <= 16u) {
-                    ne = oi->n_edges;
-                    pt0 = oi->first_pt;
-                }
-            }
-        }
-        g_geom[k] = (uint32_t)__builtin_amdgcn_readfirstlane((int)geom);
-        g_arena[k] = (uint32_t)__builtin_amdgcn_readfirstlane((int)arena);
-        g_ne[k] = (uint32_t)__builtin_amdgcn_readfirstlane((int)ne);
-        g_pt0[k] = (uint32_t)__builtin_amdgcn_readfirstlane((int)pt0);
-        g_base[k + 1] = g_base[k] + (g_geom[k] >> 24);
-    }
-    const uint32_t n_slots = g_base[FILL_GROUP];
-    if (n_slots == 0u) return;
+    if (fblk >= n_pass) return;
     sh.rowfill[lane] = 0u;
     sh.diff[lane] = 0;
     if (lane == 0u) sh.diff[64] = 0;
     __syncthreads();
-    for (uint32_t t0 = 0; t0 < n_slots; t0 += 4u) {
-        const uint32_t t = t0 + (lane >> OSMT_SUB_H_LOG2);
-        const bool row_valid = t < n_slots;
-        uint32_t my_k = 0u;
-#pragma unroll
-        for (uint32_t k = 1; k < FILL_GROUP; ++k)
-            if (t >= g_base[k] && g_base[k] < n_slots) my_k = k;
-        uint32_t geom = g_geom[0], arena = g_arena[0], base = g_base[0];
-#pragma unroll
-        for (uint32_t k = 1; k < FILL_GROUP; ++k)
-            if (my_k == k) {
-                geom = g_geom[k];
-                arena = g_arena[k];
-                base = g_base[k];
-            }
-        const uint32_t my_o = o_first + my_k;
-        const uint32_t sr0 = geom & 255u, c0 = (geom >> 8) & 255u, ncols = row_valid ? (geom >> 16) & 255u : 0u;
-        const uint32_t sr = sr0 + (t - base);
+    for (uint32_t pass = fblk; pass < n_pass; pass += n_fblk) {
+        const uint32_t q = lane >> OSMT_SUB_H_LOG2;
+        const uint4 ds = reinterpret_cast<const uint4*>(g_slots)[(size_t)pass * OSMT_FILL_PASS_SLOTS + q];
+        const uint32_t my_o = ds.x, geom = ds.z;
+        const uint32_t sr = osmt_fill_slot_sr(geom), c0 = osmt_fill_slot_c0(geom), ncols = osmt_fill_slot_ncols(geom);
+        const bool row_valid = ncols != 0u;
         const int32_t y = (int32_t)(sr * SUBH + (lane & (SUBH - 1u)));
         uint32_t row_hit = 0u;
+        uint32_t s_op[4], s_geom[4];
+#pragma unroll
+        for (uint32_t k = 0; k < 4u; ++k) {
+            s_op[k] = (uint32_t)__builtin_amdgcn_readlane((int)ds.x, (int)(k * SUBH));
+            s_geom[k] = (uint32_t)__builtin_amdgcn_readlane((int)ds.z, (int)(k * SUBH));
+        }
 
         uint32_t w0 = 0u, ww = 64u;
         while (w0 < 64u) {
@@ -1122,44 +1131,21 @@
             bool overflow = false;
             bool pooled = true;
 #pragma unroll
-            for (uint32_t k = 0; k < FILL_GROUP; ++k) {
-                const uint32_t s_lo = max(g_base[k], t0), s_hi = min(g_base[k + 1], t0 + 4u);
-                if (s_lo < s_hi && max((s_lo - t0) * SUBH, w0) < min((s_hi - t0) * SUBH, w0 + ww) && g_ne[k] == 0xFFFFFFFFu) pooled = false;
-            }
+            for (uint32_t k = 0; k < 4u; ++k)
+                if (s_geom[k] != 0u && !osmt_fill_slot_simple(s_geom[k]) && max(k * SUBH, w0) < min((k + 1u) * SUBH, w0 + ww)) pooled = false;
             if (pooled) {
-                uint32_t kq[4] = {0xFFu, 0xFFu, 0xFFu, 0xFFu}, nq = 0u;
-#pragma unroll
-                for (uint32_t q = 0; q < FILL_GROUP; ++q)
-                    if (max(g_base[q], t0) < min(g_base[q + 1], t0 + 4u)) {
-                        if (nq == 0u) kq[0] = q;
-                        if (nq == 1u) kq[1] = q;
-                        if (nq == 2u) kq[2] = q;
-                        if (nq == 3u) kq[3] = q;
-                        ++nq;
-                    }
-                const uint32_t qi = lane >> 4, e = lane & 15u;
-                const uint32_t k = qi == 0u ? kq[0] : (qi == 1u ? kq[1] : (qi == 2u ? kq[2] : kq[3]));
-                uint32_t kbase = g_base[0], kend = k == 0u ? g_base[1] : 0u, kgeom = g_geom[0], kne = k == 0u ? g_ne[0] : 0u, kpt0 = g_pt0[0];
-#pragma unroll
-                for (uint32_t q = 1; q < FILL_GROUP; ++q)
-                    if (k == q) {
-                        kbase = g_base[q];
-                        kend = g_base[q + 1];
-                        kgeom = g_geom[q];
-                        kne = g_ne[q];
-                        kpt0 = g_pt0[q];
-                    }
-                const uint32_t s_lo = max(kbase, t0), s_hi = min(kend, t0 + 4u);
+                const uint32_t e = lane & (SUBH - 1u);
+                const uint32_t kne = osmt_fill_slot_simple(geom) ? osmt_fill_slot_edges(geom) : 0u;
                 uint32_t cnt = 0u, l0 = 0u;
                 int32_t first = 0;
                 int2 p1 = make_int2(0, 0), p2 = p1;
-                if (s_lo < s_hi && e < kne) {
-                    const uint32_t la = max((s_lo - t0) * SUBH, w0), lb = min((s_hi - t0) * SUBH, w0 + ww);
+                if (e < kne) {
+                    const uint32_t la = max(q * SUBH, w0), lb = min((q + 1u) * SUBH, w0 + ww);
                     if (la < lb) {
-                        const int32_t ybase = ((int32_t)(kgeom & 255u) + (int32_t)t0 - (int32_t)kbase) * SUBH;
+                        const int32_t ybase = ((int32_t)sr - (int32_t)q) * SUBH;
                         const int32_t ya = ybase + (int32_t)la, yb = ybase + (int32_t)lb - 1;
-                        p1 = g_pts[kpt0 + e];
-                        p2 = g_pts[kpt0 + e + 1u];
+                        p1 = g_pts[ds.w + e];
+                        p2 = g_pts[ds.w + e + 1u];
                         const int32_t ytop = min(p1.y, p2.y), ybot = max(p1.y, p2.y);
                         first = max(ytop + 1, ya);
                         const int32_t last = min(ybot, yb);
@@ -1188,13 +1174,16 @@
                 }
             } else
 #pragma unroll 1
-            for (uint32_t k = 0; k < FILL_GROUP; ++k) {
-                const uint32_t s_lo = max(g_base[k], t0), s_hi = min(g_base[k + 1], t0 + 4u);
-                if (s_lo >= s_hi) continue;
-                const uint32_t la = max((s_lo - t0) * SUBH, w0), lb = min((s_hi - t0) * SUBH, w0 + ww);
+            for (uint32_t k = 0; k < 4u;) {
+                const uint32_t o = fill_sel4(s_op, k), gk = fill_sel4(s_geom, k);
+                const uint32_t s_lo = k;
+                ++k;
+                if (gk == 0u) continue;
+                while (k < 4u && fill_sel4(s_geom, k) != 0u && fill_sel4(s_op, k) == o) ++k;
+                const uint32_t s_hi = k;
+                const uint32_t la = max(s_lo * SUBH, w0), lb = min(s_hi * SUBH, w0 + ww);
                 if (la >= lb) continue;
-                const uint32_t o = o_first + k;
-                const int32_t ybase = ((int32_t)(g_geom[k] & 255u) + (int32_t)t0 - (int32_t)g_base[k]) * SUBH;
+                const int32_t ybase = ((int32_t)osmt_fill_slot_sr(gk) - (int32_t)s_lo) * SUBH;
                 const int32_t ya = ybase + (int32_t)la, yb = ybase + (int32_t)lb - 1;
                 const osmt_op* __restrict__ op = &g_ops[o];
                 const uint32_t ring_off = op->ring_off, n_rings = op->n_rings;
@@ -1265,7 +1254,7 @@
                     for (uint32_t c = 0; c < ncols; ++c) {
                         const int32_t x0 = (int32_t)((c0 + c) * SUB);
                         const uint32_t m = fill_row_streaming(g_rings, g_pts, op->ring_off, op->n_rings, y, x0, x0 + SUB - 1);
-                        g_fmask[((size_t)arena + (size_t)(sr - sr0) * ncols + c) * SUBH + (lane & (SUBH - 1u))] = m;
+                        g_fmask[(size_t)ds.y + c * SUBH + (lane & (SUBH - 1u))] = m;
                         if (m) row_hit |= 1u << (c0 + c);
                     }
                 }
@@ -1333,7 +1322,7 @@
                                 m |= bits << (uint32_t)(from - x0);
                             }
                         }
-                        g_fmask[((size_t)arena + (size_t)(sr - sr0) * ncols + c) * SUBH + (lane & (SUBH - 1u))] = m;
+                        g_fmask[(size_t)ds.y + c * SUBH + (lane & (SUBH - 1u))] = m;
                         if (m) row_hit |= 1u << (c0 + c);
                     }
                 }
@@ -1457,7 +1446,9 @@
                                                uint32_t scale, uint32_t sub_rows, uint32_t* __restrict__ g_submask,
                                                uint32_t* __restrict__ g_fmask,
                                                osmt_srec* __restrict__ g_srec, uint2* __restrict__ g_skey, const uint32_t* __restrict__ g_op_job,
-                                               uint32_t* __restrict__ g_cnt, const osmt_vseg* __restrict__ g_vseg) {
+                                               uint32_t* __restrict__ g_cnt, const osmt_vseg* __restrict__ g_vseg,
+                                               const osmt_fill_slot* __restrict__ g_slots, const unsigned long long* __restrict__ g_slot_cursor,
+                                               unsigned long long slot_cap) {
     __shared__ union {
         FillShared fill;
         StrokeBinShared bin;
@@ -1474,8 +1465,8 @@
         stroke_bin_body(shu.bin, idx, threadIdx.x, g_info, n_vsegs, scale, sub_rows, g_submask,
                         g_srec, g_skey, g_op_job, g_cnt, g_vseg);
     else
-        fill_rows_body(shu.fill, idx, threadIdx.x, g_ops, n_ops, g_info, g_rings, g_pts, g_op_blk, g_blk, scale, sub_rows, g_submask, g_fmask,
-                       g_op_job, g_cnt);
+        fill_rows_body(shu.fill, idx, roles.n_fblk, osmt_fill_pass_count(*g_slot_cursor, slot_cap), threadIdx.x, g_ops, g_slots, g_rings, g_pts,
+                       g_op_blk, g_blk, scale, sub_rows, g_submask, g_fmask, g_op_job, g_cnt);
 }
 
 #ifndef OSMT_V_SUBLIST_THREADS
@@ -2441,11 +2432,12 @@
         hipLaunchKernelGGL(k_opinfo, dim3((a.n_ops + OPINFO_THREADS * OPINFO_WAVES - 1u) / (OPINFO_THREADS * OPINFO_WAVES)),
                            dim3(OPINFO_THREADS * OPINFO_WAVES), 0, st, a);
     if (a.fmask_cap == 0 && a.srec_cap == 0) return hipGetLastError();
-    const osmt_prebin_map roles = osmt_prebin_map_make(osmt_prebin_n_vblk(a.n_vsegs, OSMT_BIN_SEGS), (a.n_ops + FILL_GROUP - 1u) / FILL_GROUP);
-    if (a.n_ops)
-        hipLaunchKernelGGL(k_prebin, dim3(roles.n_vblk + roles.n_fgrp), dim3(64), 0, st, a.ops, a.n_ops, a.info, a.rings, a.pts,
+    const uint32_t n_vblk = osmt_prebin_n_vblk(a.n_vsegs, OSMT_BIN_SEGS);
+    const osmt_prebin_map roles = osmt_prebin_map_make(n_vblk, a.n_fill_pass ? (a.n_fill_pass + FILL_BLOCK_PASSES - 1u) / FILL_BLOCK_PASSES : (a.n_ops + 1u) / 2u);
+    if (a.n_ops && roles.n_vblk + roles.n_fblk)
+        hipLaunchKernelGGL(k_prebin, dim3(roles.n_vblk + roles.n_fblk), dim3(64), 0, st, a.ops, a.n_ops, a.info, a.rings, a.pts,
                            a.op_blk, a.blk, a.n_vsegs, roles,
-                           a.scale, a.sub_rows, a.submask, a.fmask, a.srec, a.skey, a.op_job, a.cnt, a.vseg);
+                           a.scale, a.sub_rows, a.submask, a.fmask, a.srec, a.skey, a.op_job, a.cnt, a.vseg, a.slots, a.cursors + 3, a.slot_cap);
     if (a.n_jobs && (a.fold_max_ops == 0u || a.max_job_ops > a.fold_max_ops)) {
         const uint32_t Wt = OSMT_TILE_SIZE * a.scale;
         unsigned long long* const lcur = reinterpret_cast<unsigned long long*>(
diff --git a/osm_renderer_amd/csrc/osmt_prebin_roles.h b/osm_renderer_amd/csrc/osmt_prebin_roles.h
--- a/osm_renderer_amd/csrc/osmt_prebin_roles.h
+++ b/osm_renderer_amd/csrc/osmt_prebin_roles.h
@@ -24,7 +24,7 @@
 #endif
 
 struct osmt_prebin_map {
-    uint32_t n_vblk, n_fgrp;
+    uint32_t n_vblk, n_fblk;
     uint64_t magic;
 };
 
@@ -32,11 +32,11 @@
     return n_vsegs / bin_segs + (n_vsegs % bin_segs ? 1u : 0u);
 }
 
-OSMT_HD osmt_prebin_map osmt_prebin_map_make(uint32_t n_vblk, uint32_t n_fgrp) {
+OSMT_HD osmt_prebin_map osmt_prebin_map_make(uint32_t n_vblk, uint32_t n_fblk) {
     osmt_prebin_map m;
     m.n_vblk = n_vblk;
-    m.n_fgrp = n_fgrp;
-    const uint64_t T = (uint64_t)n_vblk + n_fgrp;
+    m.n_fblk = n_fblk;
+    const uint64_t T = (uint64_t)n_vblk + n_fblk;
     m.magic = T ? ~(uint64_t)0 / T : 0u;
     return m;
 }
@@ -51,7 +51,7 @@
 
 OSMT_HD uint32_t osmt_prebin_role(const osmt_prebin_map m, uint32_t b, uint32_t* idx) {
 #if OSMT_V_PREBIN_INTERLEAVE
-    const uint64_t T = (uint64_t)m.n_vblk + m.n_fgrp;
+    const uint64_t T = (uint64_t)m.n_vblk + m.n_fblk;
     const uint64_t x = (uint64_t)b * m.n_vblk;
     uint64_t s = osmt_mulhi64(x, m.magic);
     uint64_t r = x - s * T;
```

After: 1.490 million tiles/s (median of 6 runs). 1.8% higher.
